# XiYe20/NPVP

Hardware: AMD Instinct MI355X
Metric: predictor train frames/sec (higher is better)
Workload: dtype f32 (two-term fp16 split of amax-scaled operands, 3 MFMAs per product, fp32 accumulate: fp32-grade; small GEMMs: three-term bf16 split)

## Files before the change

### include/npvp_hip.h

```cpp
#ifndef NPVP_HIP_H
#define NPVP_HIP_H
#include <stddef.h>
#ifdef __cplusplus
extern "C" {
#endif

typedef void* npvp_stream_t;

int npvp_version(void);
const char* npvp_last_error(void);
long long npvp_launch_count(void);
void* npvp_stream_create_low_priority(int* least, int* greatest);
int npvp_stream_destroy(void* stream);
void* npvp_event_create(void);
int npvp_event_record(void* event, void* stream);
float npvp_event_elapsed_ms(void* event0, void* event1);
int npvp_event_destroy(void* event);

long long npvp_graph_node_counts(void* graph, long long* counts, long long* memset_bytes, int max_memsets);

long long npvp_gemm_workspace_bytes(int M, int N, int K);
int npvp_gemm_kernel_id(int a_kc, int b_kc, int M, int N, int K, int precision, int has_planes);
int npvp_gemm_route(int a_kc, int b_kc, int M, int N, int K, int precision, int has_planes, int plain_epilogue, int* out4);
int npvp_gemm_f32(int a_kc, int b_kc, int M, int N, int K, const float* A, long long lda, const float* B, long long ldb,
                  float* C, long long ldc, const float* bias, int act, const float* aux_in, float* aux_out,
                  const float* residual, long long ldr, float drop_p, int drop_mode, int drop_g1, int drop_g2,
                  const unsigned long long* seed, unsigned int salt, float alpha, int precision, float* colsum_a,
                  const void* b_pre, int accumulate, float* rowstats, const float* a_amax, const float* b_amax,
                  float* c_amax, unsigned int* range_flag, float adrop_p, int adrop_g1, int adrop_g2, unsigned int adrop_salt,
                  void* workspace, long long ws_bytes, npvp_stream_t stream);
int npvp_frame_stats_finalize(const float* part, int parts_per_frame, float values_per_part, float* mean, float* rstd,
                              int frames, float eps, npvp_stream_t stream);
int npvp_split_weight(const float* w, long long ld, int N, int K, void* F, void* D, npvp_stream_t stream);
int npvp_split_weights_batched(const void* desc, int count, npvp_stream_t stream);
int npvp_amax(const float* x, long long rows, long long cols, long long ld, float* slot, npvp_stream_t stream);

typedef struct npvp_reduce_job {
  const float* ws; float* out; long long ldc; int M, N, splits, accum; float alpha; int blocks; const float* cs_part; float* cs_out;
} npvp_reduce_job_t;
int npvp_wgrad_f16_chainable(int M, int N, int K);
long long npvp_wgrad_f16_chain_workspace_bytes(int M, int N, int K);
int npvp_wgrad_f16_chained(int M, int N, int K, const float* dy, long long lda, const float* x, long long ldb, float* dw,
                           long long ldc, float* db, int accumulate, const float* a_amax, const float* b_amax,
                           unsigned int* range_flag, float adrop_p, int adrop_g1, int adrop_g2, unsigned int adrop_salt,
                           const unsigned long long* seed, const void* prev_job, void* my_job, void* workspace,
                           long long ws_bytes, npvp_stream_t stream);
int npvp_splitk_reduce_job(const void* job, npvp_stream_t stream);
int npvp_splitk_reduce_multi(const void* jobs, int n, npvp_stream_t stream);
int npvp_linear_bwd_f16_takes(int R, int N, int K);
int npvp_linear_bwd_f16(int R, int N, int K, const float* dy, long long ldy, const float* dy_amax, const void* w_planes_d,
                        const float* w_amax, float* dx, long long ldx, int act, const float* aux_in, const float* residual,
                        long long ldr, float drop_p, int drop_mode, int drop_g1, int drop_g2, unsigned int drop_salt, float* dx_amax,
                        const float* x, long long ldxx, const float* x_amax, float* dw, long long ldw, float* db,
                        unsigned int* range_flag, float adrop_p, int adrop_g1, int adrop_g2, unsigned int adrop_salt,
                        const unsigned long long* seed, const void* prev_job, void* my_job, void* workspace, long long ws_bytes,
                        npvp_stream_t stream);
int npvp_split_weight_f16(const float* w, long long ld, int N, int K, void* F, void* D, float* amax_slot, npvp_stream_t stream);
int npvp_split_weights_f16(const void* desc, int count, void* amax_table, long long amax_bytes, npvp_stream_t stream);

int npvp_layernorm_fwd(const float* x, const float* w, const float* b, float* y, float* mean, float* rstd, long long rows,
                       int C, float eps, int relu, float* y_amax, npvp_stream_t stream);
long long npvp_layernorm_bwd_workspace_bytes(long long rows, int C);
int npvp_layernorm_bwd(const float* dy, const float* x, const float* w, const float* b, const float* mean,
                       const float* rstd, float* dx, float* dw, float* db, long long rows, int C, int relu,
                       const float* dres ,
                       int accumulate , float* dx_amax,
                       void* workspace, long long ws_bytes, npvp_stream_t stream);
int npvp_layernorm_bwd_reduce(const void* workspace, float* dw, float* db, long long rows, int C, int accumulate,
                              npvp_stream_t stream);

int npvp_layernorm_bwd_reduce_job(const void* workspace, float* dw, float* db, long long rows, int C, int accumulate, void* job);
int npvp_frameln_act_bwd_reduce_job(const void* workspace, float* dw, float* db, int frames, int per_frame, int accumulate, void* job);
int npvp_mlpdw_mid_bwd_reduce_job(const void* workspace, float* gw, float* gb, int frames, int Ch, void* job);
int npvp_sum_rows_multi(const void* jobs, int n, npvp_stream_t stream);

int npvp_layernorm_nchw_fwd(const float* x, const float* w, const float* b, float* out_nchw, float* mean, float* rstd, int frames,
                            int P, int C, float eps, int relu, npvp_stream_t stream);

int npvp_frame_stats(const float* x, const float* add, float* mean, float* rstd, int frames, int T, int per_frame,
                     float eps, npvp_stream_t stream);
int npvp_posfuse_fwd(const float* x, const float* add, const float* beta, const float* gamma, float* y, float* mean,
                     float* rstd, int N, int T, int per_frame, float eps, float* y_amax, npvp_stream_t stream);
int npvp_ln_posfuse_fwd(const float* x, const float* lw, const float* lb, float ln_eps, float* y1, float* ln_mean, float* ln_rstd,
                        const float* add, const float* beta, const float* gamma, float* fused, float* pf_mean, float* pf_rstd,
                        int N, int T, int P, int C, float pf_eps, float* y1_amax, float* fused_amax, npvp_stream_t stream);
int npvp_posfuse_bwd_fused(int N, int T, int per_frame);
int npvp_posfuse_bwd(const float* dy, const float* x, const float* add, const float* gamma, const float* mean,
                     const float* rstd, float* du, float* dyxh, float* dbeta, float* dgamma, int N, int T, int per_frame,
                     int accumulate, void* workspace, long long ws_bytes , npvp_stream_t stream);

int npvp_posfuse_instance_fwd(const float* x, const float* add, const float* beta, const float* gamma, float* y, float* mean,
                              float* rstd, int N, int T, int P, int C, float eps, float* y_amax, npvp_stream_t stream);
int npvp_posfuse_instance_bwd(const float* dy, const float* x, const float* add, const float* gamma, const float* mean,
                              const float* rstd, float* du, float* dyxh, int N, int T, int P, int C, npvp_stream_t stream);

int npvp_frameln_act_fwd(const float* h, const float* mean, const float* rstd, const float* w, const float* b,
                         const float* res, float* out, int frames, int per_frame, float drop_p, unsigned int salt,
                         float dp_p, unsigned int dp_salt, int frames_per_sample, const unsigned long long* seed,
                         float* out_amax, npvp_stream_t stream);
long long npvp_frameln_act_bwd_workspace_bytes(int frames, int per_frame);
int npvp_frameln_act_bwd(const float* dout, const float* h, const float* mean, const float* rstd, const float* w,
                         const float* b, float* dh, float* dw, float* db, int frames, int per_frame, float drop_p,
                         unsigned int salt, float dp_p, unsigned int dp_salt, int frames_per_sample,
                         const unsigned long long* seed, int accumulate ,
                         float* dh_amax, void* workspace, long long ws_bytes, npvp_stream_t stream);
int npvp_frameln_act_bwd_reduce(const void* workspace, float* dw, float* db, int frames, int per_frame, int accumulate,
                                npvp_stream_t stream);
int npvp_dwconv3x3(const float* a, const float* wt, const float* bias, float* out, int frames, int H, int W, int Ch,
                   int flip, npvp_stream_t stream);
int npvp_dwconv3x3_stats(const float* a, const float* wt, const float* bias, float* out, float* mean, float* rstd, int frames,
                         int H, int W, int Ch, float eps, void* workspace, long long ws_bytes, npvp_stream_t stream);
int npvp_mlpdw_mid_fwd(const float* h1, const float* mean1, const float* rstd1, const float* w1n, const float* b1n,
                       const float* wt, const float* bias, float* h2, float* mean2, float* rstd2, int frames, int H, int W,
                       int Ch, float eps, void* workspace, long long ws_bytes, npvp_stream_t stream);
int npvp_mlpdw_mid_fwd_parts(const float* h1, const float* part1, int J1, float nb1, float* mean1, float* rstd1, const float* w1n,
                             const float* b1n, const float* wt, const float* bias, float* h2, float* part2, int frames, int H,
                             int W, int Ch, float eps, npvp_stream_t stream);
int npvp_frameln_act_fwd_parts(const float* h, const float* part, int J, float nb, float eps, float* mean, float* rstd,
                               const float* w, const float* b, const float* res, float* out, int frames, int per_frame,
                               float drop_p, unsigned int salt, float dp_p, unsigned int dp_salt, int frames_per_sample,
                               const unsigned long long* seed, float* out_amax, npvp_stream_t stream);
long long npvp_mlpdw_mid_bwd_workspace_bytes(int frames, int Ch);
int npvp_mlpdw_mid_bwd(const float* dh2, const float* h1, const float* mean1, const float* rstd1, const float* w1n,
                       const float* b1n, const float* wt, float* da1, float* dwt_db, float* psum, int frames, int H, int W,
                       int Ch, int accumulate, void* workspace, long long ws_bytes, npvp_stream_t stream);
int npvp_mlpdw_mid_bwd_reduce(const void* workspace, float* dwt_db, int frames, int Ch, int accumulate, npvp_stream_t stream);
int npvp_mlpdw_mid_bwd_reduce_into(const void* workspace, float* gw, float* gb, int frames, int Ch, npvp_stream_t stream);
int npvp_mlpdw_mid_bwd_n2(const float* da2, const float* h2, const float* mean2, const float* rstd2, const float* w2n,
                          const float* b2n, const float* psum2, int nparts2, float drop_p, unsigned int salt,
                          const unsigned long long* seed, const float* h1, const float* mean1, const float* rstd1,
                          const float* w1n, const float* b1n, const float* wt, float* da1, float* dwt_db, float* psum, int frames,
                          int H, int W, int Ch, int accumulate, void* workspace, long long ws_bytes, npvp_stream_t stream);
int npvp_frameln_act_bwd_pgrad(const float* dout, const float* h, const float* mean, const float* rstd, const float* w,
                               const float* b, float* psum, float* dw, float* db, int frames, int per_frame, float drop_p,
                               unsigned int salt, float dp_p, unsigned int dp_salt, int frames_per_sample,
                               const unsigned long long* seed, int accumulate, void* workspace, long long ws_bytes,
                               npvp_stream_t stream);
int npvp_frameln_act_bwd_apply(const float* dout, const float* h, const float* mean, const float* rstd, const float* w,
                               const float* b, const float* psum, int nparts, float* dh, float* dw, float* db, int frames,
                               int per_frame, int accumulate, float* dh_amax, void* workspace, long long ws_bytes,
                               npvp_stream_t stream);

int npvp_im2col3x3(const float* in, float* out, int frames, int H, int W, int C, int col2im, npvp_stream_t stream);
long long npvp_dwconv3x3_wgrad_workspace_bytes(int frames, int Ch);
int npvp_dwconv3x3_wgrad(const float* a, const float* dout, float* dwt_db, int frames, int H, int W, int Ch,
                         void* workspace, long long ws_bytes, npvp_stream_t stream);

int npvp_attn_fwd(const float* q, long long ld_q, const float* k, long long ld_k, const float* v, long long ld_v, float* o,
                  long long ld_o, int mode, int dim0, int P, int W, int ws, int Tq, int Tk, int heads, int head_dim,
                  int mask_mode, float drop_p, const unsigned long long* seed, unsigned int salt, float* o_amax,
                  npvp_stream_t stream);
int npvp_attn_bwd(const float* q, long long ld_q, const float* k, long long ld_k, const float* v, long long ld_v,
                  const float* go, long long ld_o, float* dq, long long ld_dq, float* dk, long long ld_dk, float* dv,
                  long long ld_dv, int mode, int dim0, int P, int W, int ws, int Tq, int Tk, int heads, int head_dim,
                  int mask_mode, float drop_p, const unsigned long long* seed, unsigned int salt, float* dq_amax,
                  float* dk_amax , float* dv_amax,
                  npvp_stream_t stream);
int npvp_attn_long_fwd(const float* q, long long ld_q, const float* k, long long ld_k, const float* v, long long ld_v, float* o,
                       long long ld_o, int mode, int dim0, int P, int W, int ws, int Tq, int Tk, int heads, int head_dim,
                       int mask_mode, float drop_p, const unsigned long long* seed, unsigned int salt, float* o_amax,
                       npvp_stream_t stream);
long long npvp_attn_long_bwd_workspace_bytes(int mode, int dim0, int P, int W, int ws, int Tq, int Tk, int heads);
int npvp_attn_long_bwd(const float* q, long long ld_q, const float* k, long long ld_k, const float* v, long long ld_v,
                       const float* go, long long ld_o, float* dq, long long ld_dq, float* dk, long long ld_dk, float* dv,
                       long long ld_dv, int mode, int dim0, int P, int W, int ws, int Tq, int Tk, int heads, int head_dim,
                       int mask_mode, float drop_p, const unsigned long long* seed, unsigned int salt, float* dq_amax,
                       float* dk_amax , float* dv_amax, void* workspace, long long ws_bytes,
                       npvp_stream_t stream);

int npvp_drop_apply(const float* x, float* out, long long rows, int ncols, float p, int mode, int g1, int g2,
                    const unsigned long long* seed, unsigned int salt, float* out_amax, npvp_stream_t stream);
int npvp_transpose(const float* in, float* out, int batch, int R, int C, npvp_stream_t stream);
int npvp_dwtb_accumulate(const float* dwtb, float* gw, float* gb, int C, npvp_stream_t stream);
int npvp_dwtb_build(const float* w, const float* b, float* wtb, int C, npvp_stream_t stream);
int npvp_reduce_mid(const float* in, float* out, int A, int B, long long Cc, float scale, int accumulate, npvp_stream_t stream);
int npvp_broadcast_mid(const float* in, float* out, int A, int B, long long Cc, float scale, npvp_stream_t stream);

long long npvp_colsum_workspace_bytes(long long rows, int N);
int npvp_colsum(const float* x, long long rows, int N, long long ld, float* out, int accumulate ,
                void* workspace, long long ws_bytes, npvp_stream_t stream);

int npvp_l1_mean(const float* a, const float* b, long long n, float lam, float* out, void* workspace, long long ws_bytes,
                 npvp_stream_t stream);
int npvp_l1_mean_bwd(const float* a, const float* b, long long n, const float* gout, float lam, float* da, npvp_stream_t stream);
int npvp_sum_all(const float* x, long long n, float* out, void* workspace, long long ws_bytes, npvp_stream_t stream);

int npvp_grad_norm_clip(const float* g, long long n, float max_norm, float* out2, void* workspace, long long ws_bytes,
                        npvp_stream_t stream);
int npvp_adamw_step(float* p, float* g, float* m, float* v, long long n, const float* hyper, float beta1, float beta2,
                    float eps, float weight_decay, const float* clip, long long clip_begin, long long clip_end,
                    int write_back_grad, npvp_stream_t stream);

long long npvp_sqdiff_workspace_bytes(int N, long long per_image);
int npvp_sqdiff_per_image(const float* x, const float* y, int N, long long per_image, float data_range, float scale, float* out,
                          void* workspace, long long ws_bytes, npvp_stream_t stream);
long long npvp_ssim_workspace_bytes(int N, int C, int H, int W);
int npvp_ssim_per_image(const float* img1, const float* img2, int N, int C, int H, int W, const float* taps ,
                        int window_size, float* out, void* workspace, long long ws_bytes, npvp_stream_t stream);

int npvp_u8hwc_to_f32chw(const void* src_u8, float* dst, long long frames, int H, int W, int C, const float* mean,
                         const float* std, npvp_stream_t stream);

int npvp_bias_act(const float* x, const float* bias, const float* residual, float* out, long long outer, long long inner, int C,
                  int layout, int act, npvp_stream_t stream);
int npvp_act_bwd(const float* g, const float* y, float* dx, long long n, int act, npvp_stream_t stream);

int npvp_bn_workspace_bytes(int C);
int npvp_bn_stats(const float* x, long long outer, long long inner, int C, int layout, double* sums, void* workspace, long long ws_bytes,
                  npvp_stream_t stream);
int npvp_bn_act_apply(const float* x, const float* w, const float* b, const float* residual, const double* sums, long long count,
                      float eps, float momentum, float* running_mean, float* running_var, long long outer, long long inner, int C,
                      int layout, int act, float* y, float* mean, float* rstd, npvp_stream_t stream);
int npvp_bn_act_bwd(const float* g, const float* x, const float* mean, const float* rstd, const float* w, const float* b, long long outer,
                    long long inner, int C, int layout, int act, int train, float* dx, float* dw, float* db, void* workspace,
                    long long ws_bytes, npvp_stream_t stream);
int npvp_bn_act_apply_sync(const float* x, const float* w, const float* b, const float* residual, const double* stat, float eps,
                           float momentum, float* running_mean, float* running_var, long long outer, long long inner, int C, int layout,
                           int act, float* y, float* mean, float* rstd, npvp_stream_t stream);
int npvp_bn_bwd_sums(const float* g, const float* x, const float* mean, const float* rstd, const float* w, const float* b, long long outer,
                     long long inner, int C, int layout, int act, double* sums, float* dw, float* db, void* workspace, long long ws_bytes,
                     npvp_stream_t stream);
int npvp_bn_act_bwd_apply(const float* g, const float* x, const float* mean, const float* rstd, const float* w, const float* b,
                          const double* sums, const double* count, long long outer, long long inner, int C, int layout, int act, float* dx,
                          npvp_stream_t stream);
// ... 26 lines not shown
```

### npvp_amd/_lib.py

```python
import ctypes
import os

_HERE = os.path.dirname(os.path.abspath(__file__))
LIB_PATH = os.path.join(_HERE, "libnpvp_hip.so")

c_int, c_ll, c_f, c_u, c_p = ctypes.c_int, ctypes.c_longlong, ctypes.c_float, ctypes.c_uint, ctypes.c_void_p

SIGNATURES = {
    "npvp_version": (c_int, []),
    "npvp_last_error": (ctypes.c_char_p, []),
    "npvp_launch_count": (c_ll, []),
    "npvp_dp_unique_id": (c_int, [c_p]),
    "npvp_dp_init": (c_int, [c_int, c_int, c_p]),
    "npvp_dp_world": (c_int, []),
    "npvp_dp_rank": (c_int, []),
    "npvp_dp_allreduce_async": (c_int, [c_p, c_ll, c_p]),
    "npvp_dp_wait": (c_int, [c_p]),
    "npvp_dp_finalize": (c_int, []),
    "npvp_stream_create_low_priority": (c_p, [c_p, c_p]),
    "npvp_stream_destroy": (c_int, [c_p]),
    "npvp_event_create": (c_p, []),
    "npvp_event_record": (c_int, [c_p, c_p]),
    "npvp_event_elapsed_ms": (c_f, [c_p, c_p]),
    "npvp_event_destroy": (c_int, [c_p]),
    "npvp_graph_node_counts": (c_ll, [c_p, c_p, c_p, c_int]),
    "npvp_gemm_workspace_bytes": (c_ll, [c_int, c_int, c_int]),
    "npvp_gemm_kernel_id": (c_int, [c_int, c_int, c_int, c_int, c_int, c_int, c_int]),
    "npvp_gemm_route": (c_int, [c_int, c_int, c_int, c_int, c_int, c_int, c_int, c_int, c_p]),
    "npvp_gemm_f32": (c_int, [c_int, c_int, c_int, c_int, c_int, c_p, c_ll, c_p, c_ll, c_p, c_ll, c_p, c_int, c_p, c_p,
                              c_p, c_ll, c_f, c_int, c_int, c_int, c_p, c_u, c_f, c_int, c_p, c_p, c_int, c_p, c_p, c_p, c_p, c_p,
                              c_f, c_int, c_int, c_u, c_p, c_ll, c_p]),
    "npvp_amax": (c_int, [c_p, c_ll, c_ll, c_ll, c_p, c_p]),
    "npvp_wgrad_f16_chainable": (c_int, [c_int, c_int, c_int]),
    "npvp_wgrad_f16_chain_workspace_bytes": (c_ll, [c_int, c_int, c_int]),
    "npvp_wgrad_f16_chained": (c_int, [c_int, c_int, c_int, c_p, c_ll, c_p, c_ll, c_p, c_ll, c_p, c_int, c_p, c_p, c_p, c_f, c_int, c_int,
                                       c_u, c_p, c_p, c_p, c_p, c_ll, c_p]),
    "npvp_splitk_reduce_job": (c_int, [c_p, c_p]),
    "npvp_splitk_reduce_multi": (c_int, [c_p, c_int, c_p]),
    "npvp_linear_bwd_f16_takes": (c_int, [c_int, c_int, c_int]),
    "npvp_linear_bwd_f16": (c_int, [c_int, c_int, c_int, c_p, c_ll, c_p, c_p, c_p, c_p, c_ll, c_int, c_p, c_p, c_ll, c_f, c_int, c_int, c_int,
                                    c_u, c_p, c_p, c_ll, c_p, c_p, c_ll, c_p, c_p, c_f, c_int, c_int, c_u, c_p, c_p, c_p, c_p, c_ll, c_p]),
    "npvp_split_weight_f16": (c_int, [c_p, c_ll, c_int, c_int, c_p, c_p, c_p, c_p]),
    "npvp_split_weights_f16": (c_int, [c_p, c_int, c_p, c_ll, c_p]),
    "npvp_frame_stats_finalize": (c_int, [c_p, c_int, c_f, c_p, c_p, c_int, c_f, c_p]),
    "npvp_split_weight": (c_int, [c_p, c_ll, c_int, c_int, c_p, c_p, c_p]),
    "npvp_split_weights_batched": (c_int, [c_p, c_int, c_p]),
    "npvp_layernorm_fwd": (c_int, [c_p, c_p, c_p, c_p, c_p, c_p, c_ll, c_int, c_f, c_int, c_p, c_p]),
    "npvp_layernorm_bwd_workspace_bytes": (c_ll, [c_ll, c_int]),
    "npvp_layernorm_bwd": (c_int, [c_p, c_p, c_p, c_p, c_p, c_p, c_p, c_p, c_p, c_ll, c_int, c_int, c_p, c_int, c_p, c_p, c_ll, c_p]),
    "npvp_layernorm_bwd_reduce": (c_int, [c_p, c_p, c_p, c_ll, c_int, c_int, c_p]),
    "npvp_layernorm_bwd_reduce_job": (c_int, [c_p, c_p, c_p, c_ll, c_int, c_int, c_p]),
    "npvp_frameln_act_bwd_reduce_job": (c_int, [c_p, c_p, c_p, c_int, c_int, c_int, c_p]),
    "npvp_mlpdw_mid_bwd_reduce_job": (c_int, [c_p, c_p, c_p, c_int, c_int, c_p]),
    "npvp_sum_rows_multi": (c_int, [c_p, c_int, c_p]),
    "npvp_layernorm_nchw_fwd": (c_int, [c_p, c_p, c_p, c_p, c_p, c_p, c_int, c_int, c_int, c_f, c_int, c_p]),
    "npvp_frameln_act_bwd_reduce": (c_int, [c_p, c_p, c_p, c_int, c_int, c_int, c_p]),
    "npvp_frame_stats": (c_int, [c_p, c_p, c_p, c_p, c_int, c_int, c_int, c_f, c_p]),
    "npvp_posfuse_fwd": (c_int, [c_p, c_p, c_p, c_p, c_p, c_p, c_p, c_int, c_int, c_int, c_f, c_p, c_p]),
    "npvp_posfuse_instance_fwd": (c_int, [c_p, c_p, c_p, c_p, c_p, c_p, c_p, c_int, c_int, c_int, c_int, c_f, c_p, c_p]),
    "npvp_posfuse_instance_bwd": (c_int, [c_p, c_p, c_p, c_p, c_p, c_p, c_p, c_p, c_int, c_int, c_int, c_int, c_p]),
    "npvp_ln_posfuse_fwd": (c_int, [c_p, c_p, c_p, c_f, c_p, c_p, c_p, c_p, c_p, c_p, c_p, c_p, c_p, c_int, c_int, c_int, c_int, c_f,
                                    c_p, c_p, c_p]),
    "npvp_posfuse_bwd_fused": (c_int, [c_int, c_int, c_int]),
    "npvp_posfuse_bwd": (c_int, [c_p, c_p, c_p, c_p, c_p, c_p, c_p, c_p, c_p, c_p, c_int, c_int, c_int, c_int, c_p, c_ll, c_p]),
    "npvp_frameln_act_fwd": (c_int, [c_p, c_p, c_p, c_p, c_p, c_p, c_p, c_int, c_int, c_f, c_u, c_f, c_u, c_int, c_p, c_p, c_p]),
    "npvp_frameln_act_bwd_workspace_bytes": (c_ll, [c_int, c_int]),
    "npvp_frameln_act_bwd": (c_int, [c_p, c_p, c_p, c_p, c_p, c_p, c_p, c_p, c_p, c_int, c_int, c_f, c_u, c_f, c_u, c_int,
                                     c_p, c_int, c_p, c_p, c_ll, c_p]),
    "npvp_dwconv3x3": (c_int, [c_p, c_p, c_p, c_p, c_int, c_int, c_int, c_int, c_int, c_p]),
    "npvp_dwconv3x3_stats": (c_int, [c_p, c_p, c_p, c_p, c_p, c_p, c_int, c_int, c_int, c_int, c_f, c_p, c_ll, c_p]),
    "npvp_mlpdw_mid_fwd": (c_int, [c_p, c_p, c_p, c_p, c_p, c_p, c_p, c_p, c_p, c_p, c_int, c_int, c_int, c_int, c_f, c_p, c_ll, c_p]),
    "npvp_mlpdw_mid_fwd_parts": (c_int, [c_p, c_p, c_int, c_f, c_p, c_p, c_p, c_p, c_p, c_p, c_p, c_p, c_int, c_int, c_int, c_int, c_f, c_p]),
    "npvp_frameln_act_fwd_parts": (c_int, [c_p, c_p, c_int, c_f, c_f, c_p, c_p, c_p, c_p, c_p, c_p, c_int, c_int, c_f, c_u, c_f, c_u, c_int,
                                           c_p, c_p, c_p]),
    "npvp_mlpdw_mid_bwd_workspace_bytes": (c_ll, [c_int, c_int]),
    "npvp_mlpdw_mid_bwd": (c_int, [c_p, c_p, c_p, c_p, c_p, c_p, c_p, c_p, c_p, c_p, c_int, c_int, c_int, c_int, c_int, c_p, c_ll, c_p]),
    "npvp_mlpdw_mid_bwd_reduce": (c_int, [c_p, c_p, c_int, c_int, c_int, c_p]),
    "npvp_mlpdw_mid_bwd_reduce_into": (c_int, [c_p, c_p, c_p, c_int, c_int, c_p]),
    "npvp_mlpdw_mid_bwd_n2": (c_int, [c_p, c_p, c_p, c_p, c_p, c_p, c_p, c_int, c_f, c_u, c_p, c_p, c_p, c_p, c_p, c_p, c_p, c_p, c_p,
                                      c_p, c_int, c_int, c_int, c_int, c_int, c_p, c_ll, c_p]),
    "npvp_frameln_act_bwd_pgrad": (c_int, [c_p, c_p, c_p, c_p, c_p, c_p, c_p, c_p, c_p, c_int, c_int, c_f, c_u, c_f, c_u, c_int,
                                           c_p, c_int, c_p, c_ll, c_p]),
    "npvp_frameln_act_bwd_apply": (c_int, [c_p, c_p, c_p, c_p, c_p, c_p, c_p, c_int, c_p, c_p, c_p, c_int, c_int, c_int, c_p, c_p, c_ll, c_p]),
    "npvp_im2col3x3": (c_int, [c_p, c_p, c_int, c_int, c_int, c_int, c_int, c_p]),
    "npvp_dwconv3x3_wgrad_workspace_bytes": (c_ll, [c_int, c_int]),
    "npvp_dwconv3x3_wgrad": (c_int, [c_p, c_p, c_p, c_int, c_int, c_int, c_int, c_p, c_ll, c_p]),
    "npvp_attn_fwd": (c_int, [c_p, c_ll, c_p, c_ll, c_p, c_ll, c_p, c_ll, c_int, c_int, c_int, c_int, c_int, c_int, c_int,
                              c_int, c_int, c_int, c_f, c_p, c_u, c_p, c_p]),
    "npvp_attn_bwd": (c_int, [c_p, c_ll, c_p, c_ll, c_p, c_ll, c_p, c_ll, c_p, c_ll, c_p, c_ll, c_p, c_ll, c_int, c_int,
                              c_int, c_int, c_int, c_int, c_int, c_int, c_int, c_int, c_f, c_p, c_u, c_p, c_p, c_p, c_p]),
    "npvp_attn_long_fwd": (c_int, [c_p, c_ll, c_p, c_ll, c_p, c_ll, c_p, c_ll, c_int, c_int, c_int, c_int, c_int, c_int, c_int,
                                   c_int, c_int, c_int, c_f, c_p, c_u, c_p, c_p]),
    "npvp_attn_long_bwd_workspace_bytes": (c_ll, [c_int, c_int, c_int, c_int, c_int, c_int, c_int, c_int]),
    "npvp_attn_long_bwd": (c_int, [c_p, c_ll, c_p, c_ll, c_p, c_ll, c_p, c_ll, c_p, c_ll, c_p, c_ll, c_p, c_ll, c_int, c_int,
                                   c_int, c_int, c_int, c_int, c_int, c_int, c_int, c_int, c_f, c_p, c_u, c_p, c_p, c_p, c_p, c_ll, c_p]),
    "npvp_drop_apply": (c_int, [c_p, c_p, c_ll, c_int, c_f, c_int, c_int, c_int, c_p, c_u, c_p, c_p]),
    "npvp_transpose": (c_int, [c_p, c_p, c_int, c_int, c_int, c_p]),
    "npvp_dwtb_accumulate": (c_int, [c_p, c_p, c_p, c_int, c_p]),
    "npvp_dwtb_build": (c_int, [c_p, c_p, c_p, c_int, c_p]),
    "npvp_reduce_mid": (c_int, [c_p, c_p, c_int, c_int, c_ll, c_f, c_int, c_p]),
    "npvp_broadcast_mid": (c_int, [c_p, c_p, c_int, c_int, c_ll, c_f, c_p]),
    "npvp_colsum_workspace_bytes": (c_ll, [c_ll, c_int]),
    "npvp_colsum": (c_int, [c_p, c_ll, c_int, c_ll, c_p, c_int, c_p, c_ll, c_p]),
    "npvp_grad_norm_clip": (c_int, [c_p, c_ll, c_f, c_p, c_p, c_ll, c_p]),
    "npvp_l1_mean": (c_int, [c_p, c_p, c_ll, c_f, c_p, c_p, c_ll, c_p]),
    "npvp_l1_mean_bwd": (c_int, [c_p, c_p, c_ll, c_p, c_f, c_p, c_p]),
    "npvp_sum_all": (c_int, [c_p, c_ll, c_p, c_p, c_ll, c_p]),
    "npvp_adamw_step": (c_int, [c_p, c_p, c_p, c_p, c_ll, c_p, c_f, c_f, c_f, c_f, c_p, c_ll, c_ll, c_int, c_p]),
    "npvp_sqdiff_workspace_bytes": (c_ll, [c_int, c_ll]),
    "npvp_sqdiff_per_image": (c_int, [c_p, c_p, c_int, c_ll, c_f, c_f, c_p, c_p, c_ll, c_p]),
    "npvp_ssim_workspace_bytes": (c_ll, [c_int, c_int, c_int, c_int]),
    "npvp_u8hwc_to_f32chw": (c_int, [c_p, c_p, c_ll, c_int, c_int, c_int, c_p, c_p, c_p]),
    "npvp_bias_act": (c_int, [c_p, c_p, c_p, c_p, c_ll, c_ll, c_int, c_int, c_int, c_p]),
    "npvp_act_bwd": (c_int, [c_p, c_p, c_p, c_ll, c_int, c_p]),
    "npvp_bn_workspace_bytes": (c_int, [c_int]),
    "npvp_bn_stats": (c_int, [c_p, c_ll, c_ll, c_int, c_int, c_p, c_p, c_ll, c_p]),
    "npvp_bn_act_apply": (c_int, [c_p, c_p, c_p, c_p, c_p, c_ll, c_f, c_f, c_p, c_p, c_ll, c_ll, c_int, c_int, c_int, c_p, c_p, c_p, c_p]),
    "npvp_bn_act_bwd": (c_int, [c_p, c_p, c_p, c_p, c_p, c_p, c_ll, c_ll, c_int, c_int, c_int, c_int, c_p, c_p, c_p, c_p, c_ll, c_p]),
    "npvp_bn_act_apply_sync": (c_int, [c_p, c_p, c_p, c_p, c_p, c_f, c_f, c_p, c_p, c_ll, c_ll, c_int, c_int, c_int, c_p, c_p, c_p, c_p]),
    "npvp_bn_bwd_sums": (c_int, [c_p, c_p, c_p, c_p, c_p, c_p, c_ll, c_ll, c_int, c_int, c_int, c_p, c_p, c_p, c_p, c_ll, c_p]),
    "npvp_bn_act_bwd_apply": (c_int, [c_p, c_p, c_p, c_p, c_p, c_p, c_p, c_p, c_ll, c_ll, c_int, c_int, c_int, c_p, c_p]),
    "npvp_reflect_pad": (c_int, [c_p, c_p, c_int, c_int, c_int, c_int, c_int, c_int, c_int, c_p]),
    "npvp_nonlocal_attn_fwd": (c_int, [c_p, c_ll, c_p, c_ll, c_p, c_ll, c_p, c_ll, c_p, c_int, c_int, c_int, c_int, c_int, c_p]),
    "npvp_nonlocal_attn_bwd": (c_int, [c_p, c_ll, c_p, c_ll, c_p, c_ll, c_p, c_ll, c_p, c_p, c_p, c_ll, c_p, c_ll, c_p, c_ll, c_int, c_int,
                                       c_int, c_int, c_int, c_p]),
    "npvp_nonlocal_attn_grid_fwd": (c_int, [c_p, c_ll, c_p, c_ll, c_p, c_ll, c_p, c_ll, c_p, c_int, c_int, c_int, c_int, c_int, c_p]),
    "npvp_nonlocal_attn_grid_bwd": (c_int, [c_p, c_ll, c_p, c_ll, c_p, c_ll, c_p, c_ll, c_p, c_p, c_p, c_ll, c_p, c_ll, c_p, c_ll, c_int,
                                            c_int, c_int, c_int, c_int, c_p]),
    "npvp_ssim_per_image": (c_int, [c_p, c_p, c_int, c_int, c_int, c_int, c_p, c_int, c_p, c_p, c_ll, c_p]),
}

_lib = None


def lib():
    global _lib
    if _lib is None:
        if not os.path.exists(LIB_PATH):
            raise RuntimeError(
                f"{LIB_PATH} is missing - the HIP extension has not been built. Run "
                "`python -c 'import __graft_entry__ as g; g.build()'` (or `python npvp_amd/build.py`). "
                "npvp_amd has no CPU fallback.")
        L = ctypes.CDLL(LIB_PATH, mode=os.RTLD_NOW)
        bound = _Bound()
        for name, (res, args) in SIGNATURES.items():
            fn = getattr(L, name)
            fn.restype, fn.argtypes = res, args
            setattr(bound, name, fn)
        bound._cdll = L
        bound._fast = 0
        if os.environ.get("NPVP_FASTCALL", "1") == "1":
            try:
                from . import _npvp_fast as F
            except ImportError as e:
                import warnings
                warnings.warn(f"npvp_amd._npvp_fast is not built ({e}): every call goes through ctypes (same kernels, more host time)")
            else:
                for name in SIGNATURES:
                    f = getattr(F, name, None)
                    if f is not None:
                        setattr(bound, name, f)
                        bound._fast += 1
        _lib = bound
    return _lib


# ... 9 lines not shown
```

### npvp_amd/csrc/gemm.h

```cpp
#pragma once
#include <type_traits>
#include "common.h"

namespace npvp {

typedef float f32x16 __attribute__((ext_vector_type(16)));
typedef __bf16 bf16x8 __attribute__((ext_vector_type(8)));
typedef __bf16 bf16x4 __attribute__((ext_vector_type(4)));

struct ReduceJob {
  const float* ws; float* out; long long ldc; int M, N, splits, accum; float alpha; int blocks; const float* cs_part; float* cs_out;
};

struct GemmParams {
  const float* A; const float* B; float* C;
  const float* bias;
  const float* residual;
  float* aux_out;
  const float* aux_in;
  float* rowstats;
  float* colsum;
  const unsigned long long* seed;
  long long lda, ldb, ldc, ldr;
  int M, N, K;
  int act;
  DropSpec drop;
  DropSpec adrop;
  int tiles_m, tiles_n;
  int splits;
  float alpha;
  const void* b_pre;
  long long b_pre_plane;
  int colgroups;
  int accum;
  const float* a_amax; const float* b_amax; float* c_amax;
  unsigned int* range_flag;
  ReduceJob prev;
};

__device__ __forceinline__ void splitk_reduce_body(const ReduceJob& j, int bid, int nblocks, float& cmax) {
  const long long total4 = (long long)j.M * j.N / 4, cs4 = j.cs_out ? j.M / 4 : 0;
  for (long long i = (long long)bid * 256 + threadIdx.x; i < total4 + cs4; i += (long long)nblocks * 256) {
    if (i >= total4) {
      const long long e = (i - total4) * 4;
      float4 s = make_float4(0.f, 0.f, 0.f, 0.f);
      for (int zz = 0; zz < j.splits; ++zz) {
        const float4 v = ld4(j.cs_part + (long long)zz * j.M + e);
        s.x += v.x; s.y += v.y; s.z += v.z; s.w += v.w;
      }
      if (j.accum) { const float4 o = ld4(j.cs_out + e); s.x += o.x; s.y += o.y; s.z += o.z; s.w += o.w; }
      st4(j.cs_out + e, s);
      continue;
    }
    const long long e = i * 4;
    const int m = (int)(e / j.N), n = (int)(e - (long long)m * j.N);
    float4 s = make_float4(0.f, 0.f, 0.f, 0.f);
    for (int zz = 0; zz < j.splits; ++zz) {
      const float4 v = ld4(j.ws + (long long)zz * j.M * j.N + e);
      s.x += v.x; s.y += v.y; s.z += v.z; s.w += v.w;
    }
    s.x *= j.alpha; s.y *= j.alpha; s.z *= j.alpha; s.w *= j.alpha;
    if (j.accum) { const float4 o = ld4(j.out + (long long)m * j.ldc + n); s.x += o.x; s.y += o.y; s.z += o.z; s.w += o.w; }
    st4(j.out + (long long)m * j.ldc + n, s);
    cmax = amax4(cmax, s);
  }
}

__device__ __forceinline__ void store_colsum(const GemmParams& p, long long idx, float v) {
  p.colsum[idx] = (p.accum && p.splits == 1) ? p.colsum[idx] + v : v;
}

constexpr int EPI_LD = 36;
constexpr int EPI_FLOATS = 32 * EPI_LD;

__device__ __forceinline__ void epi_transpose(const f32x16& acc, float* scr, int lane, float4 (&v)[4]) {
  const int r = lane & 31, h = lane >> 5;
#pragma unroll
  for (int g = 0; g < 16; ++g) scr[(((g & 3) + 8 * (g >> 2)) + 4 * h) * EPI_LD + r] = acc[g];
  const int rr = lane >> 3, cq = lane & 7;
#pragma unroll
  for (int k = 0; k < 4; ++k) v[k] = *reinterpret_cast<const float4*>(scr + (rr + 8 * k) * EPI_LD + 4 * cq);
}

__device__ __forceinline__ float4 f4_mad(const float4& a, float s, const float4& b) {
  return make_float4(a.x * s + b.x, a.y * s + b.y, a.z * s + b.z, a.w * s + b.w);
}
__device__ __forceinline__ void f4_add(float4& a, const float4& b) { a.x += b.x; a.y += b.y; a.z += b.z; a.w += b.w; }

template <int I, int N, class F>
__device__ __forceinline__ void static_for(F&& f) {
  if constexpr (I < N) {
    f(std::integral_constant<int, I>{});
    static_for<I + 1, N>(f);
  }
}

__device__ __forceinline__ float4 epilogue_row_scales(const GemmParams& p, unsigned long long seed, int row0, int lane) {
  float4 sc = make_float4(1.f, 1.f, 1.f, 1.f);
  if (p.drop.thresh && p.drop.mode != 0) {
    const int r = row0 + (lane >> 3);
    sc.x = drop_spec_scale(p.drop, seed, r, 0, 1); sc.y = drop_spec_scale(p.drop, seed, r + 8, 0, 1);
    sc.z = drop_spec_scale(p.drop, seed, r + 16, 0, 1); sc.w = drop_spec_scale(p.drop, seed, r + 24, 0, 1);
  }
  return sc;
}

template <bool CHECK>
__device__ __forceinline__ void epilogue_rows(const GemmParams& p, float4 (&v)[4], int row0, int col0, int lane, int z,
                                              unsigned long long seed, float& cmax, float4 rowsc, float alpha) {
  const int rb = row0 + (lane >> 3), col = col0 + 4 * (lane & 7);
// ... 206 lines not shown
```

### npvp_amd/csrc/gemm.hip

```cpp
#include "gemm.h"
#include "partials.h"
#include <type_traits>

namespace npvp {

constexpr int BM = 128, BN = 128, BK = 32, GEMM_THREADS = 256;

template <bool KC> struct Stager;

template <> struct Stager<true> {
  static constexpr int LD = 129;
  float4 r[4];
  __device__ __forceinline__ void load(const float* src, long long ld, int row0, int nrows, int k0) {
    const int t = threadIdx.x;
    const int kc = (t & 7) * 4;
#pragma unroll
    for (int i = 0; i < 4; ++i) {
      const int row = row0 + (t >> 3) + 32 * i;
      r[i] = (row < nrows) ? ld4(src + (long long)row * ld + k0 + kc) : make_float4(0.f, 0.f, 0.f, 0.f);
    }
  }
  __device__ __forceinline__ void store(float* s) const {
    const int t = threadIdx.x;
    const int kc = (t & 7) * 4;
// ... 413 lines not shown
  NPVP_CHECK_ARG(N > 0 && K > 0 && N % 8 == 0 && K % 8 == 0 && ld % 4 == 0, "split_weight: N, K must be multiples of 8");
  NPVP_CHECK_ARG(((uintptr_t)w % 16) == 0, "split_weight: w must be 16-byte aligned");
  const long long total = (long long)N * K / 8;
  int blocks = (int)((total + 255) / 256); if (blocks > 4096) blocks = 4096;
  if (F) { NPVP_LAUNCH(split_weight_fwd_kernel, dim3(blocks), dim3(256), 0, stream, w, ld, N, K, (__bf16*)F); NPVP_CHECK_LAUNCH(); }
  if (D) { NPVP_LAUNCH(split_weight_dgrad_kernel, dim3(blocks), dim3(256), 0, stream, w, ld, N, K, (__bf16*)D); NPVP_CHECK_LAUNCH(); }
  return NPVP_OK;
}

extern "C" int npvp_split_weights_batched(const void* desc, int count, hipStream_t stream) {
  NPVP_CHECK_ARG(desc && count > 0, "split_weights_batched: empty table");
  NPVP_LAUNCH(split_weights_batched_kernel, dim3(128, count), dim3(256), 0, stream, (const SplitDesc*)desc);
  NPVP_CHECK_LAUNCH();
  return NPVP_OK;
}

struct GemmFacts {
  int a_kc, b_kc, M, N, K, precision;
  bool planes;
  bool plain;
  bool amax;
  bool rowstats;
  long long ws_bytes;
};
struct GemmPlan {
  int id, variant, splits, steps;
  bool planes;
};

static GemmPlan plan_gemm(const GemmFacts& f) {
  const int M = f.M, N = f.N, K = f.K;
  const bool want_h = f.precision == 6;
  const int precision = want_h ? 4 : f.precision;
  int s128 = pick_splits(M, N, K);
  if (s128 > 1 && (!f.plain || f.ws_bytes < npvp_gemm_workspace_bytes(M, N, K))) s128 = 1;
  const bool planes_ok = f.planes && f.a_kc && K % 16 == 0 && N % 8 == 0;
  const bool wgrad = !f.a_kc && !f.b_kc && f.plain && !f.rowstats;
  auto fits = [&](int s) { return s == 1 || (s > 1 && f.ws_bytes >= splitk_workspace_bytes(s, M, N)); };
  GemmPlan pl = {precision == 0 ? 0 : 1, 0, s128, 0, false};
  int v = 0, s = 0;
  if (want_h && planes_ok && f.amax && (v = gemm_f16_variant(M, N, K)) != 0) {
    pl.id = v == 1 ? 5 : 7; pl.variant = v; pl.splits = 1; pl.planes = true;
  } else if (want_h && wgrad && f.amax && fits(s = f16_wgrad_splits(M, N, K))) {
    pl.id = 6; pl.splits = s;
  } else if (!want_h && precision == 4 && planes_ok && s128 == 1 && (v = wide_variant(M, N, K)) != 0) {
    pl.id = v == 1 ? 2 : 4; pl.variant = v; pl.planes = true;
  } else if (precision == 4 && wgrad && fits(s = wide_wgrad_splits(M, N, K))) {
    pl.id = 3; pl.splits = s;
  } else {
    pl.planes = !want_h && precision == 4 && planes_ok && s128 == 1 && !f.rowstats;
  }
  pl.steps = K / pl.splits / (precision == 0 ? BK : 16);
  return pl;
}

static GemmPlan plan_query(int a_kc, int b_kc, int M, int N, int K, int precision, int has_planes, bool plain) {
  return plan_gemm(GemmFacts{a_kc, b_kc, M, N, K, precision, has_planes != 0, plain, true, false, npvp_gemm_workspace_bytes(M, N, K)});
}

extern "C" int npvp_gemm_kernel_id(int a_kc, int b_kc, int M, int N, int K, int precision, int has_planes) {
  return plan_query(a_kc, b_kc, M, N, K, precision, has_planes, true).id;
}

extern "C" int npvp_gemm_route(int a_kc, int b_kc, int M, int N, int K, int precision, int has_planes, int plain_epilogue, int* out4) {
  NPVP_CHECK_ARG(out4 && M > 0 && N > 0 && K > 0, "gemm_route: empty problem or no result array");
  NPVP_CHECK_ARG(precision == 0 || precision == 4 || precision == 5 || precision == 6, "gemm_route: precision must be 0, 4, 5 or 6");
  NPVP_CHECK_ARG(K % BK == 0 && M % 4 == 0 && N % 4 == 0 && !(a_kc == 0 && b_kc == 1), "gemm_route: not a problem npvp_gemm_f32 accepts");
  const GemmPlan r = plan_query(a_kc, b_kc, M, N, K, precision, has_planes, plain_epilogue != 0);
  out4[0] = r.id; out4[1] = r.variant; out4[2] = r.splits; out4[3] = r.steps;
  return NPVP_OK;
}

static int finish_splitk(const GemmParams& p, float* C, long long ldc, float* colsum_a, hipStream_t stream) {
  const long long total4 = (long long)p.M * p.N / 4;
  int blocks = (int)((total4 + 255) / 256); if (blocks > 2048) blocks = 2048;
  const bool cs_here = colsum_a && ((uintptr_t)colsum_a % 16) == 0;
  NPVP_LAUNCH(splitk_reduce_kernel, dim3(blocks), dim3(256), 0, stream, (const float*)p.C, C, p.M, p.N, ldc, p.splits, p.alpha,
              p.accum, cs_here ? (const float*)p.colsum : nullptr, cs_here ? colsum_a : nullptr, p.c_amax);
  NPVP_CHECK_LAUNCH();
  if (!colsum_a || cs_here) return NPVP_OK;
  return finish_partials(make_partials(p.colsum, 0, p.splits, p.splits, p.M, colsum_a, p.accum).job, 0, stream, "gemm: column-sum reduce launch failed");
}

extern "C" int npvp_gemm_f32(int a_kc, int b_kc, int M, int N, int K, const float* A, long long lda, const float* B,
                             long long ldb, float* C, long long ldc, const float* bias, int act, const float* aux_in,
                             float* aux_out, const float* residual, long long ldr, float drop_p, int drop_mode,
                             int drop_g1, int drop_g2, const unsigned long long* seed, unsigned int salt, float alpha,
                             int precision, float* colsum_a, const void* b_pre, int accumulate, float* rowstats,
                             const float* a_amax, const float* b_amax, float* c_amax, unsigned int* range_flag,
                             float adrop_p, int adrop_g1, int adrop_g2, unsigned int adrop_salt,
                             void* workspace, long long ws_bytes, hipStream_t stream) {
  NPVP_CHECK_ARG(M > 0 && N > 0 && K > 0, "gemm: empty problem");
  NPVP_CHECK_ARG(precision == 0 || precision == 4 || precision == 5 || precision == 6,
                 "gemm: precision must be 0 (exact fp32-input MFMA), 4 (three-term bf16 split, 6 MFMAs per product: "
                 "fp32-grade), 5 (two-term bf16 split, 3 MFMAs per product, ~2^-16) or 6 (two-term fp16 split with amax-scaled "
                 "operands, 3 MFMAs per product: fp32-grade; shapes it does not take run as 4)");
  const bool want_h = precision == 6;
  NPVP_CHECK_ARG(K % BK == 0, "gemm: K must be a multiple of 32");
  NPVP_CHECK_ARG(M % 4 == 0 && N % 4 == 0, "gemm: M and N must be multiples of 4");
  NPVP_CHECK_ARG(((uintptr_t)A % 16) == 0 && ((uintptr_t)B % 16) == 0 && ((uintptr_t)C % 16) == 0, "gemm: pointers must be 16-byte aligned");
  NPVP_CHECK_ARG(lda % 4 == 0 && ldb % 4 == 0, "gemm: lda/ldb must be multiples of 4 floats");
  NPVP_CHECK_ARG(ldc % 4 == 0 && (!residual || (ldr % 4 == 0 && ((uintptr_t)residual % 16) == 0)) && (!bias || ((uintptr_t)bias % 16) == 0) &&
                 (!aux_in || ((uintptr_t)aux_in % 16) == 0) && (!aux_out || ((uintptr_t)aux_out % 16) == 0),
                 "gemm: ldc / ldr must be multiples of 4 floats and bias / aux / residual 16-byte aligned (float4 epilogue)");
  NPVP_CHECK_ARG(!(a_kc == 0 && b_kc == 1), "gemm: (a_kc=0,b_kc=1) is not used by the path");
  NPVP_CHECK_ARG((act != 3 && act != 4) || aux_in, "gemm: act 3/4 need aux_in");
  NPVP_CHECK_ARG(drop_p >= 0.f && drop_p < 1.f, "gemm: dropout p out of range");
  NPVP_CHECK_ARG(drop_p == 0.f || seed, "gemm: dropout needs a device seed");
  NPVP_CHECK_ARG(!colsum_a || a_kc == 0, "gemm: colsum_a is the column sum of a [K][M] operand (a_kc = 0)");
  NPVP_CHECK_ARG(!b_pre || ((uintptr_t)b_pre % 16) == 0, "gemm: b_pre must be 16-byte aligned");

  NPVP_CHECK_ARG(adrop_p >= 0.f && adrop_p < 0.5f, "gemm: adrop_p must be in [0, 0.5) (the masked operand must stay inside its amax scale)");
  NPVP_CHECK_ARG(adrop_p == 0.f || (seed && want_h && adrop_g1 > 0 && adrop_g2 > 0 && (a_kc || adrop_g1 % 16 == 0)),
                 "gemm: adrop needs precision 6, a device seed and (for a weight gradient) groups of a multiple of 16 rows");
  NPVP_CHECK_ARG(!rowstats || ((precision == 4 || want_h) && a_kc && b_kc && M % 64 == 0 && N % 128 == 0 && act == 0 && !aux_out && !residual &&
                               drop_p == 0.f && !accumulate),
                 "gemm: rowstats needs the default (bf16x6) forward layout, M % 64 == 0, N % 128 == 0 and a bias-only epilogue");

  const bool plain = !bias && act == 0 && !aux_out && !residual && drop_p == 0.f;
  const GemmPlan plan = plan_gemm(GemmFacts{a_kc, b_kc, M, N, K, precision, b_pre != nullptr, plain,
                                            a_amax && b_amax, rowstats != nullptr, workspace ? ws_bytes : 0});
  NPVP_CHECK_ARG(adrop_p == 0.f || plan.id >= 5, "gemm: adrop was requested but this shape does not run on the fp16 kernels (npvp_gemm_kernel_id tells)");

  GemmParams p;
  p.A = A; p.B = B; p.bias = bias; p.residual = residual; p.aux_out = aux_out; p.aux_in = aux_in;
  p.seed = seed; p.lda = lda; p.ldb = ldb; p.ldr = ldr; p.M = M; p.N = N; p.act = act;
  p.drop = make_drop_spec(drop_p, salt, drop_mode, drop_g1, drop_g2);
  p.adrop = make_drop_spec(adrop_p, adrop_salt, 1, adrop_g1, adrop_g2);
  p.alpha = alpha;
  p.rowstats = rowstats;
  p.a_amax = a_amax; p.b_amax = b_amax; p.c_amax = c_amax; p.range_flag = range_flag;
  p.prev = ReduceJob{};
  p.accum = accumulate ? 1 : 0;
  p.b_pre = plan.planes ? b_pre : nullptr;
  p.b_pre_plane = (long long)N * K;
  p.splits = plan.splits;
  if (plan.splits > 1) aim_at_workspace(p, K, plan.splits, workspace, colsum_a != nullptr);
  else { p.K = K; p.C = C; p.ldc = ldc; p.colsum = colsum_a; }
  p.tiles_m = (M + BM - 1) / BM; p.tiles_n = (N + BN - 1) / BN;
  p.colgroups = (plan.id <= 1 && plan.splits == 1) ? pick_colgroups((long long)N * K * 4, p.tiles_m, p.tiles_n) : 1;

  const dim3 grid(p.tiles_m * p.tiles_n, plan.splits), block(GEMM_THREADS);
  switch (plan.id) {
    case 5: case 7: launch_gemm_f16(p, plan.variant, stream); break;
    case 6: launch_gemm_wgrad_f16(p, stream); break;
    case 2: case 4: launch_gemm_wide(p, plan.variant, stream); break;
    case 3: launch_gemm_wgrad_wide(p, stream); break;
    case 0:
      if (a_kc && b_kc) NPVP_LAUNCH((gemm_f32_kernel<true, true>), grid, block, 0, stream, p);
      else if (a_kc) NPVP_LAUNCH((gemm_f32_kernel<true, false>), grid, block, 0, stream, p);
      else NPVP_LAUNCH((gemm_f32_kernel<false, false>), grid, block, 0, stream, p);
      break;
    default:
      if (precision == 5) {
        if (a_kc && b_kc) NPVP_LAUNCH((gemm_split_db_kernel<2, true, true, false>), grid, block, 0, stream, p);
        else if (a_kc) NPVP_LAUNCH((gemm_split_db_kernel<2, true, false, false>), grid, block, 0, stream, p);
        else NPVP_LAUNCH((gemm_split_db_kernel<2, false, false, false>), grid, block, 0, stream, p);
      } else if (rowstats) NPVP_LAUNCH((gemm_split_db_kernel<3, true, true, false, true>), grid, block, 0, stream, p);
      else if (plan.planes) NPVP_LAUNCH((gemm_split_db_kernel<3, true, true, true>), grid, block, 0, stream, p);
      else if (a_kc && b_kc) NPVP_LAUNCH((gemm_split_db_kernel<3, true, true, false>), grid, block, 0, stream, p);
      else if (a_kc) NPVP_LAUNCH((gemm_split_db_kernel<3, true, false, false>), grid, block, 0, stream, p);
      else NPVP_LAUNCH((gemm_split_db_kernel<3, false, false, false>), grid, block, 0, stream, p);
  }
  NPVP_CHECK_LAUNCH();
  return plan.splits > 1 ? finish_splitk(p, C, ldc, colsum_a, stream) : NPVP_OK;
}
```

### npvp_amd/csrc/gemm_f16.hip

```cpp
#include "gemm.h"
#include <cstdlib>

namespace npvp {

typedef _Float16 f16x8 __attribute__((ext_vector_type(8)));
typedef _Float16 f16x4 __attribute__((ext_vector_type(4)));
typedef __attribute__((address_space(1))) const void* gptr_t;
typedef __attribute__((address_space(3))) void* lptr_t;
typedef float f32x4 __attribute__((ext_vector_type(4)));

__device__ __forceinline__ void split_f16_scaled(const f32x4 v, const float s, f16x4& hi, f16x4& lo) {
  unsigned int h01, h23, l01, l23;
  asm("v_fma_mixlo_f16 %0, %1, %2, 0" : "=v"(h01) : "v"(v[0]), "v"(s));
  asm("v_fma_mixlo_f16 %0, %1, %2, 0" : "=v"(h23) : "v"(v[2]), "v"(s));
  asm("v_fma_mixhi_f16 %0, %1, %2, 0" : "+v"(h01) : "v"(v[1]), "v"(s));
  asm("v_fma_mixhi_f16 %0, %1, %2, 0" : "+v"(h23) : "v"(v[3]), "v"(s));
  asm("v_fma_mixlo_f16 %0, %1, %2, -%3 op_sel_hi:[0,0,1]" : "=v"(l01) : "v"(v[0]), "v"(s), "v"(h01));
  asm("v_fma_mixlo_f16 %0, %1, %2, -%3 op_sel_hi:[0,0,1]" : "=v"(l23) : "v"(v[2]), "v"(s), "v"(h23));
  asm("v_fma_mixhi_f16 %0, %1, %2, -%3 op_sel:[0,0,1] op_sel_hi:[0,0,1]" : "+v"(l01) : "v"(v[1]), "v"(s), "v"(h01));
  asm("v_fma_mixhi_f16 %0, %1, %2, -%3 op_sel:[0,0,1] op_sel_hi:[0,0,1]" : "+v"(l23) : "v"(v[3]), "v"(s), "v"(h23));
  typedef unsigned int u32x2 __attribute__((ext_vector_type(2)));
  const u32x2 hp = {h01, h23}, lp = {l01, l23};
  hi = __builtin_bit_cast(f16x4, hp);
  lo = __builtin_bit_cast(f16x4, lp);
// ... 23 lines not shown
__device__ __forceinline__ void gemm_f16_body(const GemmParams& p, char* lds, const int bid, const int nwg) {
  constexpr int NW = WM * WN, THREADS = 64 * NW;
  constexpr int BM = WM * TM * 32, BN = WN * TN * 32;
  constexpr int APASS = BM / (THREADS / 4);
  static_assert((APASS == 1 || APASS == 2) && BN % 64 == 0, "A staging: a thread stages one or two rows of the tile");
  constexpr int KGS_A = BM * 16 + 64, A_PLANE = 2 * KGS_A, A_BYTES = 2 * A_PLANE;
  constexpr int KGS_B = BN * 16, B_PLANE = 2 * KGS_B, B_BYTES = 2 * B_PLANE;
  constexpr int STAGE = A_BYTES + B_BYTES;
  constexpr int CPS = BN / 64;
  constexpr int NCHUNK = 4 * CPS, CPW = (NCHUNK + NW - 1) / NW;
  static_assert(NST == 2 || NST == 3, "two or three LDS stages");
  static_assert(gemm_f16_lds_bytes<TM, TN, WM, WN, NST>() >= NST * STAGE, "lds size formula");

  int tile_m, tile_n;
  tile_of_block_unsplit(p, nwg, bid, tile_m, tile_n);
  const int m0 = tile_m * BM, n0 = tile_n * BN;
  const int t = threadIdx.x, lane = t & 63, wave = __builtin_amdgcn_readfirstlane(t >> 6);
  const int wm = wave / WN, wn = wave % WN, r = lane & 31, h = lane >> 5;
  const int nk = p.K >> 4;
  const float sa = amax_scale(amax_slot_read(p.a_amax));
  const unsigned int cpeek = amax_peek_block(p.c_amax);

  f32x16 acc[TM][TN];

  const int quad = t & 3, rl = t >> 2;
  const char* a_base = reinterpret_cast<const char*>(p.A + (long long)m0 * p.lda);
  const unsigned int a_off0 = (unsigned int)(((long long)(min(m0 + rl, p.M - 1) - m0) * p.lda + 4 * quad) * 4);
  const unsigned int a_off1 = (unsigned int)(((long long)(min(m0 + rl + BM / 2, p.M - 1) - m0) * p.lda + 4 * quad) * 4);
  const int a_dst = (quad >> 1) * KGS_A + (quad & 1) * 8 + rl * 16;
  float sa0 = sa, sa1 = sa;
  if (p.adrop.thresh) {
    const unsigned long long aseed = *p.seed;
    sa0 *= drop_spec_scale(p.adrop, aseed, min(m0 + rl, p.M - 1), 0, 1);
    sa1 *= drop_spec_scale(p.adrop, aseed, min(m0 + rl + BM / 2, p.M - 1), 0, 1);
  }
  const char* b_base = reinterpret_cast<const char*>(p.b_pre);
  unsigned int b_off[CPW];
  int b_dst[CPW];
#pragma unroll
  for (int i = 0; i < CPW; ++i) {
    const int c = wave + NW * i;
    const int slab = c / CPS, part = c - slab * CPS, s = slab >> 1, kg = slab & 1;
    const int col = min(n0 + part * 64 + lane, p.N - 1);
    b_off[i] = (unsigned int)(((long long)s * (p.b_pre_plane >> 3) + (long long)kg * p.N + col) * 16);
    b_dst[i] = A_BYTES + s * B_PLANE + kg * KGS_B + part * 1024;
  }
  const long long b_step = 32ll * p.N;
  const unsigned int lds_u32 = (unsigned int)(size_t)((lptr_t)lds);

  const int fa_off = h * KGS_A + (wm * TM * 32 + r) * 16;
  const int fb_off = A_BYTES + h * KGS_B + (wn * TN * 32 + r) * 16;

  f32x4 ea0, ea1 = {0.f, 0.f, 0.f, 0.f}, eb0, eb1 = {0.f, 0.f, 0.f, 0.f};
#define NPVP_H_ALOAD(R0, R1, KT)                                                                           \
  { const char* ab_ = a_base + ((long long)min((KT), nk - 1) << 6);                                        \
    asm volatile("global_load_dwordx4 %0, %1, %2" : "=v"(R0) : "v"(a_off0), "s"(ab_) : "memory");          \
    if constexpr (APASS == 2) asm volatile("global_load_dwordx4 %0, %1, %2" : "=v"(R1) : "v"(a_off1), "s"(ab_) : "memory"); }
#define NPVP_H_WAIT_BUT_NEWEST(...)                                                                        \
  { if constexpr (APASS == 2) asm volatile("s_waitcnt vmcnt(2) lgkmcnt(0)" : __VA_ARGS__ :: "memory");     \
    else asm volatile("s_waitcnt vmcnt(1) lgkmcnt(0)" : __VA_ARGS__ :: "memory"); }
#define NPVP_H_WAIT_BUT_THIS_STEP(...)                                                                     \
  asm volatile("s_waitcnt vmcnt(%2) lgkmcnt(0)" : __VA_ARGS__ : "n"(CPW + APASS) : "memory");
#define NPVP_H_ASTORE(ST, V, ROWOFF)                                                     \
  { if (ROWOFF) rm1 = fmaxf(fmaxf(rm1, fmaxf(fabsf((V)[0]), fabsf((V)[1]))), fmaxf(fabsf((V)[2]), fabsf((V)[3])));  \
    else rm0 = fmaxf(fmaxf(rm0, fmaxf(fabsf((V)[0]), fabsf((V)[1]))), fmaxf(fabsf((V)[2]), fabsf((V)[3])));         \
    f16x4 hi_, lo_; split_f16_scaled((V), (ROWOFF) ? sa1 : sa0, hi_, lo_);               \
    *reinterpret_cast<f16x4*>((ST) + a_dst + (ROWOFF)) = hi_;                            \
    *reinterpret_cast<f16x4*>((ST) + A_PLANE + a_dst + (ROWOFF)) = lo_; }
#define NPVP_H_BLOAD(ST, KT)                                                             \
  { const char* bb_ = b_base + (long long)min((KT), nk - 1) * b_step;                    \
    _Pragma("unroll") for (int i_ = 0; i_ < CPW; ++i_)                                   \
      if (NCHUNK % NW == 0 || wave + NW * i_ < NCHUNK) {                                 \
        const unsigned int m0_ = lds_u32 + (unsigned int)((ST) - lds) + (unsigned int)b_dst[i_];          \
        asm volatile("s_mov_b32 m0, %0\n\ts_nop 0\n\tglobal_load_lds_dwordx4 %1, %2"                     \
                     :: "s"(m0_), "v"(b_off[i_]), "s"(bb_) : "memory", "m0"); } }
  static_assert(NCHUNK % NW == 0, "the hand-counted waits assume CPW LDS-DMA pieces per wave and step");

  __shared__ int guard_flags[NW];
  float rm0 = 0.f, rm1 = 0.f;
  bool rescued = false;
  const float zrow = 1.f;
  float rf0 = zrow, rf1 = zrow;
  const f32x16 zero16 = {0.f, 0.f, 0.f, 0.f, 0.f, 0.f, 0.f, 0.f, 0.f, 0.f, 0.f, 0.f, 0.f, 0.f, 0.f, 0.f};
  auto run_tile = [&]() __attribute__((always_inline)) {
  NPVP_H_BLOAD(lds, 0)
  NPVP_H_ALOAD(ea0, ea1, 0)
  asm volatile("s_waitcnt vmcnt(0)" : "+v"(ea0), "+v"(ea1) :: "memory");
  NPVP_H_ASTORE(lds, ea0, 0)
  if constexpr (APASS == 2) NPVP_H_ASTORE(lds, ea1, (BM / 2) * 16)
  if constexpr (NST == 3) NPVP_H_BLOAD(lds + STAGE, 1)
  NPVP_H_ALOAD(ea0, ea1, 1)
  NPVP_H_ALOAD(eb0, eb1, 2)
  NPVP_H_WAIT_BUT_NEWEST("+v"(ea0), "+v"(ea1))
  __builtin_amdgcn_s_barrier();

#define NPVP_H_STEP(KT, CUR, NXT, R0, R1, RN0, RN1) NPVP_H_STEP_(KT, CUR, NXT, NXT, R0, R1, RN0, RN1, false)
#define NPVP_H_STEP3(KT, CUR, NXT, B2, R0, R1, RN0, RN1) NPVP_H_STEP_(KT, CUR, NXT, B2, R0, R1, RN0, RN1, false)
#define NPVP_H_STEP_(KT, CUR, NXT, B2, R0, R1, RN0, RN1, FIRST)                                            \
  {                                                                                                        \
    const char* st_ = lds + (CUR) * STAGE;                                                                 \
    char* nx_ = lds + (NXT) * STAGE;                                                                       \
    NPVP_H_BLOAD(lds + (B2) * STAGE, (KT) + (NST - 1))                                                     \
    f16x8 fb_[2][TN];                                                                                      \
    _Pragma("unroll") for (int s_ = 0; s_ < 2; ++s_)                                                       \
      _Pragma("unroll") for (int j_ = 0; j_ < TN; ++j_)                                                    \
        fb_[s_][j_] = *reinterpret_cast<const f16x8*>(st_ + fb_off + s_ * B_PLANE + j_ * 512);             \
    _Pragma("unroll") for (int i_ = 0; i_ < TM; ++i_) {                                                    \
      f16x8 fa_[2];                                                                                        \
      _Pragma("unroll") for (int s_ = 0; s_ < 2; ++s_)                                                     \
        fa_[s_] = *reinterpret_cast<const f16x8*>(st_ + fa_off + s_ * A_PLANE + i_ * 512);                 \
      if (i_ == 0) { NPVP_H_ASTORE(nx_, R0, 0) if constexpr (APASS == 2) NPVP_H_ASTORE(nx_, R1, (BM / 2) * 16) } \
      if (i_ == TM - 1) { NPVP_H_ALOAD(R0, R1, (KT) + 3) }                                                 \
                                                                                 \
      _Pragma("unroll") for (int j_ = 0; j_ < TN; ++j_) acc[i_][j_] = __builtin_amdgcn_mfma_f32_32x32x16_f16(fa_[1], fb_[0][j_], (FIRST) ? zero16 : acc[i_][j_], 0, 0, 0); \
      _Pragma("unroll") for (int j_ = 0; j_ < TN; ++j_) acc[i_][j_] = __builtin_amdgcn_mfma_f32_32x32x16_f16(fa_[0], fb_[1][j_], acc[i_][j_], 0, 0, 0); \
      _Pragma("unroll") for (int j_ = 0; j_ < TN; ++j_) acc[i_][j_] = __builtin_amdgcn_mfma_f32_32x32x16_f16(fa_[0], fb_[0][j_], acc[i_][j_], 0, 0, 0); \
    }                                                                                                      \
    __builtin_amdgcn_sched_barrier(0);        \
    if constexpr (NST == 3) { NPVP_H_WAIT_BUT_THIS_STEP("+v"(RN0), "+v"(RN1)) }                            \
    else { NPVP_H_WAIT_BUT_NEWEST("+v"(RN0), "+v"(RN1)) }                                                  \
    __builtin_amdgcn_s_barrier();                                                                          \
  }

  if constexpr (NST == 2) {
  NPVP_H_STEP_(0, 0, 1, 1, ea0, ea1, eb0, eb1, true)
  int kt = 1;
  for (; kt + 1 < nk; kt += 2) {
    NPVP_H_STEP(kt, 1, 0, eb0, eb1, ea0, ea1)
    NPVP_H_STEP(kt + 1, 0, 1, ea0, ea1, eb0, eb1)
  }
  if (kt < nk) NPVP_H_STEP(kt, 1, 0, eb0, eb1, ea0, ea1)
  } else {
  NPVP_H_STEP_(0, 0, 1, 2, ea0, ea1, eb0, eb1, true)
  int kt = 1;
  for (; kt + 5 < nk; kt += 6) {
    NPVP_H_STEP3(kt, 1, 2, 0, eb0, eb1, ea0, ea1)
    NPVP_H_STEP3(kt + 1, 2, 0, 1, ea0, ea1, eb0, eb1)
    NPVP_H_STEP3(kt + 2, 0, 1, 2, eb0, eb1, ea0, ea1)
    NPVP_H_STEP3(kt + 3, 1, 2, 0, ea0, ea1, eb0, eb1)
    NPVP_H_STEP3(kt + 4, 2, 0, 1, eb0, eb1, ea0, ea1)
    NPVP_H_STEP3(kt + 5, 0, 1, 2, ea0, ea1, eb0, eb1)
  }
  if (kt < nk) NPVP_H_STEP3(kt, 1, 2, 0, eb0, eb1, ea0, ea1)
  if (kt + 1 < nk) NPVP_H_STEP3(kt + 1, 2, 0, 1, ea0, ea1, eb0, eb1)
  if (kt + 2 < nk) NPVP_H_STEP3(kt + 2, 0, 1, 2, eb0, eb1, ea0, ea1)
  if (kt + 3 < nk) NPVP_H_STEP3(kt + 3, 1, 2, 0, ea0, ea1, eb0, eb1)
  if (kt + 4 < nk) NPVP_H_STEP3(kt + 4, 2, 0, 1, eb0, eb1, ea0, ea1)
  }
  asm volatile("s_waitcnt vmcnt(0)" : "+v"(ea0), "+v"(ea1), "+v"(eb0), "+v"(eb1) :: "memory");
  if constexpr (NST == 3) __builtin_amdgcn_s_barrier();
  };
  run_tile();
  {
    rm0 = fmaxf(rm0, __shfl_xor(rm0, 1)); rm0 = fmaxf(rm0, __shfl_xor(rm0, 2));
    rm1 = fmaxf(rm1, __shfl_xor(rm1, 1)); rm1 = fmaxf(rm1, __shfl_xor(rm1, 2));
    const int et = (int)((__float_as_uint(sa) >> 23) & 0xffu);
    const int e0 = (int)((__float_as_uint(rm0) >> 23) & 0xffu), e1 = (int)((__float_as_uint(rm1) >> 23) & 0xffu);
    const int d0 = 268 - et - e0, d1 = 268 - et - e1;
    const bool ok0 = e0 >= 16 && e0 != 255 && d0 > 0 && d0 <= 120, ok1 = e1 >= 16 && e1 != 255 && d1 > 0 && d1 <= 120;
    if (block_any<NW>((ok0 && d0 >= 18) || (ok1 && d1 >= 18), guard_flags, wave)) {
      const float g0 = sa0 * pow2_recip(sa), g1 = sa1 * pow2_recip(sa);
      rf0 = ok0 ? __uint_as_float((unsigned int)(127 - d0) << 23) : 1.f;
      rf1 = ok1 ? __uint_as_float((unsigned int)(127 - d1) << 23) : 1.f;
      sa0 = (ok0 ? amax_scale(rm0) : sa) * g0;
      sa1 = (ok1 ? amax_scale(rm1) : sa) * g1;
      rescued = true;
// ... 596 lines not shown
```

### npvp_amd/csrc/norm.hip

```cpp
#include "partials.h"
#include <cstring>
#include <cstdlib>

namespace npvp {

template <int NV>
__global__ __launch_bounds__(256) void ln_fwd_kernel(const float* __restrict__ x, const float* __restrict__ w,
                                                     const float* __restrict__ b, float* __restrict__ y,
                                                     float* __restrict__ mean, float* __restrict__ rstd, long long rows,
                                                     float eps, int relu, float* __restrict__ amax) {
  constexpr int C = NV * 256;
  __shared__ float ared[4];
  const unsigned int peek = amax_peek_block(amax);
  const int lane = threadIdx.x & 63;
  float4 ww[NV], bb[NV];
#pragma unroll
  for (int i = 0; i < NV; ++i) { ww[i] = ld4(w + (i * 64 + lane) * 4); bb[i] = ld4(b + (i * 64 + lane) * 4); }
  float am = 0.f;
  for (long long row = (long long)blockIdx.x * 4 + (threadIdx.x >> 6); row < rows; row += (long long)gridDim.x * 4) {
    float4 v[NV];
    float s = 0.f;
#pragma unroll
    for (int i = 0; i < NV; ++i) {
      v[i] = ld4(x + row * C + (i * 64 + lane) * 4);
// ... 447 lines not shown
  }
  if (dbeta) {
    if (accum) { const float4 o = ld4(dbeta + (long long)t * per_frame + e); sb.x += o.x; sb.y += o.y; sb.z += o.z; sb.w += o.w; }
    st4(dbeta + (long long)t * per_frame + e, sb);
  }
  if (dgamma) {
    if (accum) { const float4 o = ld4(dgamma + (long long)t * per_frame + e); sg.x += o.x; sg.y += o.y; sg.z += o.z; sg.w += o.w; }
    st4(dgamma + (long long)t * per_frame + e, sg);
  }
}

constexpr int PFI_MAXP = 64;
__global__ __launch_bounds__(256) void posfuse_inst_fwd_kernel(const float* __restrict__ x, const float* __restrict__ add,
                                                               const float* __restrict__ beta, const float* __restrict__ gamma,
                                                               float* __restrict__ y, float* __restrict__ mean,
                                                               float* __restrict__ rstd, int T, int P, int C, float eps,
                                                               float* __restrict__ amax) {
  __shared__ float ared[4];
  const unsigned int peek = amax_peek_block(amax);
  const int c = blockIdx.x * blockDim.x + threadIdx.x;
  const long long f = blockIdx.y;
  float am = 0.f;
  if (c < C) {
    const int n = (int)(f / T), t = (int)(f - (long long)n * T);
    const float* xp = x + f * P * C + c;
    const float* ap = add ? add + (long long)n * P * C + c : nullptr;
    float u[PFI_MAXP], s = 0.f;
#pragma unroll
    for (int p = 0; p < PFI_MAXP; ++p) if (p < P) { u[p] = xp[(long long)p * C] + (ap ? ap[(long long)p * C] : 0.f); s += u[p]; }
    const float mu = s / P;
    float q = 0.f;
#pragma unroll
    for (int p = 0; p < PFI_MAXP; ++p) if (p < P) { const float d = u[p] - mu; q += d * d; }
    const float rs = rsqrtf(q / P + eps);
    mean[f * C + c] = mu; rstd[f * C + c] = rs;
    const float* bp = beta + (long long)t * P * C + c;
    const float* gp = gamma ? gamma + (long long)t * P * C + c : nullptr;
#pragma unroll
    for (int p = 0; p < PFI_MAXP; ++p) if (p < P) {
      float o = (u[p] - mu) * rs;
      if (gp) o *= 1.f + gp[(long long)p * C];
      o += bp[(long long)p * C];
      y[f * P * C + (long long)p * C + c] = o;
      am = fmaxf(am, fabsf(o));
    }
  }
  amax_slot_commit_block(amax, am, ared, peek);
}

__global__ __launch_bounds__(256) void posfuse_inst_bwd_kernel(const float* __restrict__ dy, const float* __restrict__ x,
                                                               const float* __restrict__ add, const float* __restrict__ gamma,
                                                               const float* __restrict__ mean, const float* __restrict__ rstd,
                                                               float* __restrict__ du, float* __restrict__ dyxh, int T, int P,
                                                               int C) {
  const int c = blockIdx.x * blockDim.x + threadIdx.x;
  const long long f = blockIdx.y;
  if (c >= C) return;
  const int n = (int)(f / T), t = (int)(f - (long long)n * T);
  const long long base = f * P * C + c;
  const float* ap = add ? add + (long long)n * P * C + c : nullptr;
  const float* gp = gamma ? gamma + (long long)t * P * C + c : nullptr;
  const float mu = mean[f * C + c], rs = rstd[f * C + c];
  float g[PFI_MAXP], uh[PFI_MAXP], s1 = 0.f, s2 = 0.f;
#pragma unroll
  for (int p = 0; p < PFI_MAXP; ++p) if (p < P) {
    const float d = dy[base + (long long)p * C];
    uh[p] = (x[base + (long long)p * C] + (ap ? ap[(long long)p * C] : 0.f) - mu) * rs;
    if (dyxh) dyxh[base + (long long)p * C] = d * uh[p];
    g[p] = gp ? d * (1.f + gp[(long long)p * C]) : d;
    s1 += g[p]; s2 += g[p] * uh[p];
  }
  s1 /= P; s2 /= P;
#pragma unroll
  for (int p = 0; p < PFI_MAXP; ++p) if (p < P) du[base + (long long)p * C] = rs * (g[p] - s1 - uh[p] * s2);
}

struct FlnParams {
  const float* h; const float* mean; const float* rstd; const float* w; const float* b;
  const float* res;
  const unsigned long long* seed;
  unsigned int drop_thresh; float drop_inv_keep; unsigned int salt;
  unsigned int dp_thresh; float dp_inv_keep; unsigned int dp_salt; int frames_per_sample;
  int per_frame; long long total4;
};

__device__ __forceinline__ float fln_frame_scale(const FlnParams& p, unsigned long long seed, long long f) {
  if (!p.dp_thresh) return 1.f;
  return drop_scale(seed, p.dp_salt, (unsigned long long)((unsigned int)f / (unsigned int)p.frames_per_sample), p.dp_thresh, p.dp_inv_keep);
}
__device__ __forceinline__ float fln_scale(const FlnParams& p, unsigned long long seed, float frame_scale, long long gidx) {
  if (!p.drop_thresh) return frame_scale;
  return drop_scale(seed, p.salt, (unsigned long long)gidx, p.drop_thresh, p.drop_inv_keep) * frame_scale;
}

__global__ void frameln_act_fwd_kernel(FlnParams p, float* __restrict__ out, float* __restrict__ amax) {
  const int pf4 = p.per_frame / 4;
  __shared__ float ared[16];
  const unsigned int peek = amax_peek_block(amax);
  float am = 0.f;
  const unsigned long long seed = (p.seed && (p.drop_thresh || p.dp_thresh)) ? *p.seed : 0ull;
  for (long long i = (long long)blockIdx.x * blockDim.x + threadIdx.x; i < p.total4; i += (long long)gridDim.x * blockDim.x) {
    const long long f = i / pf4;
    const int e = (int)(i - f * pf4) * 4;
    const float mu = p.mean[f], rs = p.rstd[f];
    const float fsc = fln_frame_scale(p, seed, f);
    const float4 v = ld4(p.h + f * p.per_frame + e), ww = ld4(p.w + e), bb = ld4(p.b + e);
    const long long g0 = f * p.per_frame + e;
    float4 o;
    o.x = gelu_f((v.x - mu) * rs * ww.x + bb.x) * fln_scale(p, seed, fsc, g0 + 0);
    o.y = gelu_f((v.y - mu) * rs * ww.y + bb.y) * fln_scale(p, seed, fsc, g0 + 1);
    o.z = gelu_f((v.z - mu) * rs * ww.z + bb.z) * fln_scale(p, seed, fsc, g0 + 2);
    o.w = gelu_f((v.w - mu) * rs * ww.w + bb.w) * fln_scale(p, seed, fsc, g0 + 3);
    if (p.res) { const float4 r = ld4(p.res + g0); o.x += r.x; o.y += r.y; o.z += r.z; o.w += r.w; }
    st4(out + g0, o);
    am = amax4(am, o);
  }
  amax_slot_commit_block(amax, am, ared, peek);
}

__global__ __launch_bounds__(256) void frameln_act_fwd_parts_kernel(FlnParams p, const float* __restrict__ part, int J, float nb,
                                                                    float eps, float* __restrict__ mean_out,
                                                                    float* __restrict__ rstd_out, float* __restrict__ out,
                                                                    float* __restrict__ amax) {
  __shared__ float ared[16];
  const unsigned int peek = amax_peek_block(amax);
  const int bpf = p.per_frame / 4096;
  const long long f = blockIdx.x / bpf;
  const int e0 = (blockIdx.x - (int)f * bpf) * 4096;
  const unsigned long long seed = (p.seed && (p.drop_thresh || p.dp_thresh)) ? *p.seed : 0ull;
  float mu, rs;
  frame_stats_merge(part, f, J, nb, eps, mu, rs);
  if (e0 == 0 && threadIdx.x == 0) { mean_out[f] = mu; rstd_out[f] = rs; }
  const float fsc = fln_frame_scale(p, seed, f);
  float am = 0.f;
#pragma unroll
  for (int k = 0; k < 4; ++k) {
    const int e = e0 + (k * 256 + threadIdx.x) * 4;
    const long long g0 = f * p.per_frame + e;
    const float4 v = ld4(p.h + g0), ww = ld4(p.w + e), bb = ld4(p.b + e);
    float4 o;
    o.x = gelu_f((v.x - mu) * rs * ww.x + bb.x) * fln_scale(p, seed, fsc, g0 + 0);
    o.y = gelu_f((v.y - mu) * rs * ww.y + bb.y) * fln_scale(p, seed, fsc, g0 + 1);
    o.z = gelu_f((v.z - mu) * rs * ww.z + bb.z) * fln_scale(p, seed, fsc, g0 + 2);
    o.w = gelu_f((v.w - mu) * rs * ww.w + bb.w) * fln_scale(p, seed, fsc, g0 + 3);
    if (p.res) { const float4 r = ld4(p.res + g0); o.x += r.x; o.y += r.y; o.z += r.z; o.w += r.w; }
    st4(out + g0, o);
    am = amax4(am, o);
  }
  amax_slot_commit_block(amax, am, ared, peek);
}

constexpr int FLN_PARTS = 4;
__global__ __launch_bounds__(512) void frameln_act_bwd_stats_kernel(FlnParams p, const float* __restrict__ dout,
                                                                    float* __restrict__ psum) {
  __shared__ float red[8];
  const long long f = blockIdx.x;
  const unsigned long long seed = (p.seed && (p.drop_thresh || p.dp_thresh)) ? *p.seed : 0ull;
  const float mu = p.mean[f], rs = p.rstd[f];
  const float fsc = fln_frame_scale(p, seed, f);
  float s1 = 0.f, s2 = 0.f;
  const int span = p.per_frame / FLN_PARTS, e0 = blockIdx.y * span, e1 = blockIdx.y == FLN_PARTS - 1 ? p.per_frame : e0 + span;
  for (int e = e0 + threadIdx.x * 4; e < e1; e += 512 * 4) {
    const long long g0 = f * p.per_frame + e;
    const float4 v = ld4(p.h + g0), ww = ld4(p.w + e), bb = ld4(p.b + e), d = ld4(dout + g0);
    const float hx = (v.x - mu) * rs, hy = (v.y - mu) * rs, hz = (v.z - mu) * rs, hw = (v.w - mu) * rs;
    const float gx = d.x * fln_scale(p, seed, fsc, g0 + 0) * gelu_grad_f(hx * ww.x + bb.x) * ww.x;
    const float gy = d.y * fln_scale(p, seed, fsc, g0 + 1) * gelu_grad_f(hy * ww.y + bb.y) * ww.y;
    const float gz = d.z * fln_scale(p, seed, fsc, g0 + 2) * gelu_grad_f(hz * ww.z + bb.z) * ww.z;
    const float gw = d.w * fln_scale(p, seed, fsc, g0 + 3) * gelu_grad_f(hw * ww.w + bb.w) * ww.w;
    s1 += gx + gy + gz + gw;
    s2 += gx * hx + gy * hy + gz * hz + gw * hw;
  }
  s1 = block_sum<8>(s1, red);
  s2 = block_sum<8>(s2, red);
  if (threadIdx.x == 0) { psum[(f * FLN_PARTS + blockIdx.y) * 2] = s1; psum[(f * FLN_PARTS + blockIdx.y) * 2 + 1] = s2; }
}

__global__ void frameln_act_bwd_fused_kernel(FlnParams p, const float* __restrict__ dout, const float* __restrict__ psum,
                                             float* __restrict__ dh, float* __restrict__ part, int frames,
                                             int frames_per_chunk, int nparts, float* __restrict__ amax) {
  const int e = (blockIdx.x * blockDim.x + threadIdx.x) * 4;
  __shared__ float ared[16];
  const unsigned int peek = amax_peek_block(amax);
  float am = 0.f;
  if (e >= p.per_frame) { amax_slot_commit_block(amax, am, ared, peek); return; }
  const unsigned long long seed = (p.seed && (p.drop_thresh || p.dp_thresh)) ? *p.seed : 0ull;
  const float4 ww = ld4(p.w + e), bb = ld4(p.b + e);
  float4 aw = make_float4(0.f, 0.f, 0.f, 0.f), ab = make_float4(0.f, 0.f, 0.f, 0.f);
  const int f0 = blockIdx.y * frames_per_chunk;
  const int f1 = min(frames, f0 + frames_per_chunk);
  for (long long f = f0; f < f1; ++f) {
    const long long g0 = f * p.per_frame + e;
    const float mu = p.mean[f], rs = p.rstd[f];
    const float fsc = fln_frame_scale(p, seed, f);
    float a1 = 0.f, a2 = 0.f;
    for (int j = 0; j < nparts; ++j) { a1 += psum[(f * nparts + j) * 2]; a2 += psum[(f * nparts + j) * 2 + 1]; }
    a1 /= p.per_frame; a2 /= p.per_frame;
    const float4 v = ld4(p.h + g0), d = ld4(dout + g0);
    const float hx = (v.x - mu) * rs, hy = (v.y - mu) * rs, hz = (v.z - mu) * rs, hw = (v.w - mu) * rs;
    const float dx_ = d.x * fln_scale(p, seed, fsc, g0 + 0) * gelu_grad_f(hx * ww.x + bb.x);
    const float dy_ = d.y * fln_scale(p, seed, fsc, g0 + 1) * gelu_grad_f(hy * ww.y + bb.y);
    const float dz_ = d.z * fln_scale(p, seed, fsc, g0 + 2) * gelu_grad_f(hz * ww.z + bb.z);
    const float dw_ = d.w * fln_scale(p, seed, fsc, g0 + 3) * gelu_grad_f(hw * ww.w + bb.w);
    aw.x += dx_ * hx; aw.y += dy_ * hy; aw.z += dz_ * hz; aw.w += dw_ * hw;
    ab.x += dx_; ab.y += dy_; ab.z += dz_; ab.w += dw_;
    float4 o;
    o.x = rs * (dx_ * ww.x - a1 - hx * a2); o.y = rs * (dy_ * ww.y - a1 - hy * a2);
    o.z = rs * (dz_ * ww.z - a1 - hz * a2); o.w = rs * (dw_ * ww.w - a1 - hw * a2);
    st4(dh + g0, o);
    am = amax4(am, o);
  }
  amax_slot_commit_block(amax, am, ared, peek);
  float* o = part + (long long)blockIdx.y * 2 * p.per_frame;
  st4(o + e, aw);
  st4(o + p.per_frame + e, ab);
}

__global__ __launch_bounds__(256) void frameln_act_bwd_pgrad_kernel(FlnParams p, const float* __restrict__ dout,
                                                                    float* __restrict__ psum, float* __restrict__ part, int frames,
                                                                    int frames_per_chunk) {
  __shared__ float red[4];
  const int e = (blockIdx.x * blockDim.x + threadIdx.x) * 4;
  const int nblk = gridDim.x;
  const unsigned long long seed = (p.seed && (p.drop_thresh || p.dp_thresh)) ? *p.seed : 0ull;
  const float4 ww = ld4(p.w + e), bb = ld4(p.b + e);
  float4 aw = make_float4(0.f, 0.f, 0.f, 0.f), ab = make_float4(0.f, 0.f, 0.f, 0.f);
  const int f0 = blockIdx.y * frames_per_chunk;
  const int f1 = min(frames, f0 + frames_per_chunk);
  for (long long f = f0; f < f1; ++f) {
    const long long g0 = f * p.per_frame + e;
    const float mu = p.mean[f], rs = p.rstd[f];
    const float fsc = fln_frame_scale(p, seed, f);
    const float4 v = ld4(p.h + g0), d = ld4(dout + g0);
    const float hx = (v.x - mu) * rs, hy = (v.y - mu) * rs, hz = (v.z - mu) * rs, hw = (v.w - mu) * rs;
    const float dx_ = d.x * fln_scale(p, seed, fsc, g0 + 0) * gelu_grad_f(hx * ww.x + bb.x);
    const float dy_ = d.y * fln_scale(p, seed, fsc, g0 + 1) * gelu_grad_f(hy * ww.y + bb.y);
    const float dz_ = d.z * fln_scale(p, seed, fsc, g0 + 2) * gelu_grad_f(hz * ww.z + bb.z);
    const float dw_ = d.w * fln_scale(p, seed, fsc, g0 + 3) * gelu_grad_f(hw * ww.w + bb.w);
    aw.x += dx_ * hx; aw.y += dy_ * hy; aw.z += dz_ * hz; aw.w += dw_ * hw;
    ab.x += dx_; ab.y += dy_; ab.z += dz_; ab.w += dw_;
    const float gx = dx_ * ww.x, gy = dy_ * ww.y, gz = dz_ * ww.z, gw = dw_ * ww.w;
    const float s1 = block_sum<4>((gx + gy) + (gz + gw), red);
    const float s2 = block_sum<4>((gx * hx + gy * hy) + (gz * hz + gw * hw), red);
    if (threadIdx.x == 0) { psum[(f * nblk + blockIdx.x) * 2] = s1; psum[(f * nblk + blockIdx.x) * 2 + 1] = s2; }
  }
  float* o = part + (long long)blockIdx.y * 2 * p.per_frame;
  st4(o + e, aw);
  st4(o + p.per_frame + e, ab);
}

struct SumRowsPlan { int cw, threads; };
static SumRowsPlan plan_sum_rows(const SumRowsJob& q) {
  if (q.mode == 0 && q.nb < 64 && q.ncols >= 4096 && q.ncols % 4 == 0 && q.stride % 4 == 0 && (!q.out_b || q.split % 4 == 0)
      && ((uintptr_t)q.in & 15) == 0)
    return {sum_rows_wide_cols(), 1024};
  if (q.nb >= 64 && q.ncols <= 8192) return {16, 1024};
  return {64, q.nb >= 64 ? 1024 : 256};
}

int launch_sum_rows(const SumRowsJob& q, hipStream_t stream) {
  if (q.mode != 0) return NPVP_ERR_ARG;
  const SumRowsPlan pl = plan_sum_rows(q);
  const auto kernel = pl.cw == sum_rows_wide_cols() ? sum_rows_wide_kernel : pl.cw == 16 ? sum_rows_kernel<16> : sum_rows_kernel<64>;
  NPVP_LAUNCH(kernel, dim3((q.ncols + pl.cw - 1) / pl.cw), dim3(pl.threads), 0, stream, q.in, q.out, q.nb, q.stride, q.ncols, q.accum,
              q.out_b, q.out_b ? q.split : 0);
  return hipGetLastError() == hipSuccess ? NPVP_OK : NPVP_ERR_LAUNCH;
}

struct SumRowsBatch { SumRowsJob j[SRJ_MAX]; int first[SRJ_MAX + 1]; int cw[SRJ_MAX]; int n; };

__global__ __launch_bounds__(1024) void sum_rows_multi_kernel(SumRowsBatch b) {
  __shared__ float red[1024];
  int lo = 0, hi = b.n - 1;
  while (lo < hi) { const int mid = (lo + hi + 1) >> 1; if (b.first[mid] <= (int)blockIdx.x) lo = mid; else hi = mid - 1; }
  const SumRowsJob& J = b.j[lo];
  const int CW = b.cw[lo], sh = CW == 16 ? 4 : 6;
  if (CW == sum_rows_wide_cols()) {
    sum_rows_wide(J.in, J.out, J.out_b, J.nb, J.stride, J.ncols, J.out_b ? J.split : 0, J.accum,
                  (((int)blockIdx.x - b.first[lo]) * 1024 + (int)threadIdx.x) * 4);
    return;
  }
  const int cx = threadIdx.x & (CW - 1), rl = threadIdx.x >> sh, nrl = 1024 >> sh;
  const int c = ((int)blockIdx.x - b.first[lo]) * CW + cx;
  float s = 0.f;
  if (c < J.ncols)
    for (int r = rl; r < J.nb; r += nrl) s += J.in[(long long)r * J.stride + c];
  red[rl * CW + cx] = s;
  __syncthreads();
  if (rl == 0 && c < J.ncols) {
    float t = 0.f;
    for (int i = 0; i < nrl; ++i) t += red[i * CW + cx];
    float* o;
    if (J.mode == 1) { const int tap = c / J.split, ch = c - tap * J.split; o = tap < 9 ? J.out + ch * 9 + tap : J.out_b + ch; }
    else o = (J.out_b && c >= J.split) ? J.out_b + (c - J.split) : J.out + c;
    *o = J.accum ? *o + t : t;
  }
}

static inline int ew_blocks(long long total, int threads) {
  long long b = (total + threads - 1) / threads;
  if (b > 4096) b = 4096;
  if (b < 1) b = 1;
  return (int)b;
}

static void fill_fln(FlnParams& p, const float* h, const float* mean, const float* rstd, const float* w, const float* b,
                     const float* res, int frames, int per_frame, float drop_p, unsigned int salt, float dp_p,
                     unsigned int dp_salt, int frames_per_sample, const unsigned long long* seed) {
  p.h = h; p.mean = mean; p.rstd = rstd; p.w = w; p.b = b; p.res = res; p.seed = seed;
  p.drop_thresh = drop_p > 0.f ? drop_threshold(drop_p) : 0u;
  p.drop_inv_keep = drop_p > 0.f ? 1.f / (1.f - drop_p) : 1.f;
  p.salt = salt;
  p.dp_thresh = dp_p > 0.f ? drop_threshold(dp_p) : 0u;
  p.dp_inv_keep = dp_p > 0.f ? 1.f / (1.f - dp_p) : 1.f;
  p.dp_salt = dp_salt; p.frames_per_sample = frames_per_sample > 0 ? frames_per_sample : 1;
  p.per_frame = per_frame; p.total4 = (long long)frames * per_frame / 4;
}

}

using namespace npvp;

#define LN_LAUNCH(kernel, C, ...)                                                                         \
  switch ((C) / 256) {                                                                                    \
    case 1: NPVP_LAUNCH(kernel<1>, __VA_ARGS__); break;  case 2: NPVP_LAUNCH(kernel<2>, __VA_ARGS__); break;   \
    case 3: NPVP_LAUNCH(kernel<3>, __VA_ARGS__); break;  default: NPVP_LAUNCH(kernel<4>, __VA_ARGS__); break;  \
  }

extern "C" int npvp_layernorm_fwd(const float* x, const float* w, const float* b, float* y, float* mean, float* rstd,
                                  long long rows, int C, float eps, int relu, float* amax, hipStream_t stream) {
  NPVP_CHECK_ARG(rows > 0, "layernorm: no rows");
  NPVP_CHECK_ARG(C % 256 == 0 && C >= 256 && C <= 1024, "layernorm: C must be 256, 512, 768 or 1024");
  const long long nb = (rows + 3) / 4;
  LN_LAUNCH(ln_fwd_kernel, C, dim3((unsigned)(nb > 4096 ? 4096 : nb)), dim3(256), 0, stream, x, w, b, y, mean, rstd, rows, eps, relu, amax);
  NPVP_CHECK_LAUNCH();
  return NPVP_OK;
}

static int ln_bwd_blocks(long long rows) {
  long long b = (rows + 3) / 4;
  return (int)(b > 512 ? 512 : b);
}

static Partials ln_partials(const void* ws, float* dw, float* db, long long rows, int C, int accumulate) {
  const int nb = ln_bwd_blocks(rows);
  return make_partials(ws, 0, nb, nb, 2 * C, dw, accumulate, db, C);
}

extern "C" long long npvp_layernorm_bwd_workspace_bytes(long long rows, int C) {
  return ln_partials(nullptr, nullptr, nullptr, rows, C, 0).bytes;
}

extern "C" int npvp_layernorm_bwd(const float* dy, const float* x, const float* w, const float* b, const float* mean,
                                  const float* rstd, float* dx, float* dw, float* db, long long rows, int C, int relu,
                                  const float* dres, int accumulate, float* amax, void* workspace, long long ws_bytes,
                                  hipStream_t stream) {
  NPVP_CHECK_ARG(rows > 0, "layernorm_bwd: no rows");
  NPVP_CHECK_ARG(C % 256 == 0 && C >= 256 && C <= 1024, "layernorm_bwd: C must be 256, 512, 768 or 1024");
  const Partials P = ln_partials(workspace, dw, db, rows, C, accumulate);
  NPVP_CHECK_ARG(workspace && ws_bytes >= P.bytes, "layernorm_bwd: workspace too small");
  LN_LAUNCH(ln_bwd_kernel, C, dim3(P.job.nb), dim3(256), 0, stream, dy, x, w, b, mean, rstd, dx, P.part(), rows, relu, dres, amax);
  NPVP_CHECK_LAUNCH();
  return finish_partials(P.job, accumulate, stream, "layernorm_bwd: reduce launch failed");
}

extern "C" int npvp_layernorm_bwd_reduce(const void* workspace, float* dw, float* db, long long rows, int C, int accumulate,
                                         hipStream_t stream) {
  NPVP_CHECK_ARG(workspace && dw && db && rows > 0, "layernorm_bwd_reduce: bad arguments");
  return finish_partials(ln_partials(workspace, dw, db, rows, C, accumulate).job, 0, stream, "layernorm_bwd_reduce: launch failed");
}

extern "C" int npvp_layernorm_bwd_reduce_job(const void* workspace, float* dw, float* db, long long rows, int C, int accumulate, void* job) {
  NPVP_CHECK_ARG(workspace && dw && db && rows > 0 && job, "layernorm_bwd_reduce_job: bad arguments");
  return put_job(job, ln_partials(workspace, dw, db, rows, C, accumulate).job);
}

extern "C" int npvp_sum_rows_multi(const void* jobs, int n, hipStream_t stream) {
  NPVP_CHECK_ARG(jobs && n > 0, "sum_rows_multi: no jobs");
  const SumRowsJob* J = (const SumRowsJob*)jobs;
  for (int at = 0; at < n; at += SRJ_MAX) {
    SumRowsBatch b;
    b.n = n - at < SRJ_MAX ? n - at : SRJ_MAX;
    int blocks = 0;
    for (int i = 0; i < b.n; ++i) {
      b.j[i] = J[at + i];
      NPVP_CHECK_ARG(b.j[i].in && b.j[i].out && b.j[i].nb > 0 && b.j[i].ncols > 0, "sum_rows_multi: bad job");
      b.cw[i] = plan_sum_rows(b.j[i]).cw;
      b.first[i] = blocks;
      blocks += (b.j[i].ncols + b.cw[i] - 1) / b.cw[i];
    }
    b.first[b.n] = blocks;
    NPVP_LAUNCH(sum_rows_multi_kernel, dim3(blocks), dim3(1024), 0, stream, b);
    NPVP_CHECK_LAUNCH();
  }
  return NPVP_OK;
}

extern "C" int npvp_layernorm_nchw_fwd(const float* x, const float* w, const float* b, float* out, float* mean, float* rstd,
                                       int frames, int P, int C, float eps, int relu, hipStream_t stream) {
// ... 71 lines not shown
  NPVP_CHECK_ARG(!dgamma || dyxh, "posfuse_bwd: this shape needs the dy*uhat scratch (dyxh) for dgamma");
  const long long total4 = (long long)frames * per_frame / 4;
  NPVP_LAUNCH(posfuse_bwd_apply_kernel, dim3(ew_blocks(total4, 256)), dim3(256), 0, stream, dy, x, add, gamma, mean,
                     rstd, (const float*)s1, (const float*)s2, du, dgamma ? dyxh : nullptr, T, per_frame, total4);
  NPVP_CHECK_LAUNCH();
  if (dbeta) { const int rc = npvp_reduce_mid_launch(dy, dbeta, 1, N, (long long)T * per_frame, 1.f, stream, accumulate); if (rc) return rc; }
  if (dgamma) { const int rc = npvp_reduce_mid_launch(dyxh, dgamma, 1, N, (long long)T * per_frame, 1.f, stream, accumulate); if (rc) return rc; }
  return NPVP_OK;
}

extern "C" int npvp_posfuse_instance_fwd(const float* x, const float* add, const float* beta, const float* gamma, float* y,
                                         float* mean, float* rstd, int N, int T, int P, int C, float eps, float* y_amax,
                                         hipStream_t stream) {
  NPVP_CHECK_ARG(N > 0 && T > 0 && P > 0 && P <= PFI_MAXP && C > 0, "posfuse_instance: bad shape (P <= 64)");
  NPVP_LAUNCH(posfuse_inst_fwd_kernel, dim3((C + 255) / 256, N * T), dim3(256), 0, stream, x, add, beta, gamma, y, mean,
                     rstd, T, P, C, eps, y_amax);
  NPVP_CHECK_LAUNCH();
  return NPVP_OK;
}

extern "C" int npvp_posfuse_instance_bwd(const float* dy, const float* x, const float* add, const float* gamma, const float* mean,
                                         const float* rstd, float* du, float* dyxh, int N, int T, int P, int C,
                                         hipStream_t stream) {
  NPVP_CHECK_ARG(N > 0 && T > 0 && P > 0 && P <= PFI_MAXP && C > 0, "posfuse_instance_bwd: bad shape (P <= 64)");
  NPVP_LAUNCH(posfuse_inst_bwd_kernel, dim3((C + 255) / 256, N * T), dim3(256), 0, stream, dy, x, add, gamma, mean, rstd,
                     du, dyxh, T, P, C);
  NPVP_CHECK_LAUNCH();
  return NPVP_OK;
}

extern "C" int npvp_frameln_act_fwd(const float* h, const float* mean, const float* rstd, const float* w, const float* b,
                                    const float* res, float* out, int frames, int per_frame, float drop_p,
                                    unsigned int salt, float dp_p, unsigned int dp_salt, int frames_per_sample,
                                    const unsigned long long* seed, float* amax, hipStream_t stream) {
  NPVP_CHECK_ARG(frames > 0 && per_frame % 4 == 0, "frameln_act: bad shape");
  NPVP_CHECK_ARG((drop_p == 0.f && dp_p == 0.f) || seed, "frameln_act: dropout needs a device seed");
  FlnParams p;
  fill_fln(p, h, mean, rstd, w, b, res, frames, per_frame, drop_p, salt, dp_p, dp_salt, frames_per_sample, seed);
  NPVP_LAUNCH(frameln_act_fwd_kernel, dim3(ew_blocks(p.total4, 256)), dim3(256), 0, stream, p, out, amax);
  NPVP_CHECK_LAUNCH();
  return NPVP_OK;
}

extern "C" int npvp_frameln_act_fwd_parts(const float* h, const float* part, int J, float nb, float eps, float* mean, float* rstd,
                                          const float* w, const float* b, const float* res, float* out, int frames,
                                          int per_frame, float drop_p, unsigned int salt, float dp_p, unsigned int dp_salt,
                                          int frames_per_sample, const unsigned long long* seed, float* amax, hipStream_t stream) {
  NPVP_CHECK_ARG(frames > 0 && per_frame % 4096 == 0 && part && J > 0 && nb > 0.f && mean && rstd, "frameln_act_fwd_parts: bad arguments");
  NPVP_CHECK_ARG((drop_p == 0.f && dp_p == 0.f) || seed, "frameln_act: dropout needs a device seed");
  NPVP_CHECK_ARG((long long)frames * (per_frame / 4096) < (1ll << 31), "frameln_act_fwd_parts: too many blocks");
  FlnParams p;
  fill_fln(p, h, nullptr, nullptr, w, b, res, frames, per_frame, drop_p, salt, dp_p, dp_salt, frames_per_sample, seed);
  NPVP_LAUNCH(frameln_act_fwd_parts_kernel, dim3((unsigned)((long long)frames * (per_frame / 4096))), dim3(256), 0, stream, p,
                     part, J, nb, eps, mean, rstd, out, amax);
  NPVP_CHECK_LAUNCH();
  return NPVP_OK;
}

static int fln_chunks(int frames) {
  if (frames >= 512) return 32;
  const int c = frames / 2 < 16 ? frames / 2 : 16;
  return c < 1 ? 1 : c;
}

static Partials fln_partials(const void* ws, float* dw, float* db, int frames, int per_frame, int accumulate) {
  return make_partials(ws, (long long)frames * 2 * FLN_PARTS, frames, fln_chunks(frames), 2 * per_frame, dw, accumulate, db, per_frame);
}

extern "C" long long npvp_frameln_act_bwd_workspace_bytes(int frames, int per_frame) {
  return fln_partials(nullptr, nullptr, nullptr, frames, per_frame, 0).bytes;
}

static int fln_bwd_fused(const FlnParams& p, const float* dout, const float* psum, int nparts, float* dh, const Partials& P, int frames,
                         int accumulate, float* amax, hipStream_t stream, const char* error) {
  NPVP_LAUNCH(frameln_act_bwd_fused_kernel, dim3((p.per_frame / 4 + 255) / 256, P.job.nb), dim3(256), 0, stream, p,
                     dout, psum, dh, P.part(), frames, P.per, nparts, amax);
  NPVP_CHECK_LAUNCH();
  return finish_partials(P.job, accumulate, stream, error);
}

extern "C" int npvp_frameln_act_bwd(const float* dout, const float* h, const float* mean, const float* rstd, const float* w,
                                    const float* b, float* dh, float* dw, float* db, int frames, int per_frame,
                                    float drop_p, unsigned int salt, float dp_p, unsigned int dp_salt,
                                    int frames_per_sample, const unsigned long long* seed, int accumulate, float* amax,
                                    void* workspace, long long ws_bytes, hipStream_t stream) {
  NPVP_CHECK_ARG(frames > 0 && per_frame % 4 == 0, "frameln_act_bwd: bad shape");
  const Partials P = fln_partials(workspace, dw, db, frames, per_frame, accumulate);
  NPVP_CHECK_ARG(workspace && ws_bytes >= P.bytes, "frameln_act_bwd: workspace too small");
  FlnParams p;
  fill_fln(p, h, mean, rstd, w, b, nullptr, frames, per_frame, drop_p, salt, dp_p, dp_salt, frames_per_sample, seed);
  NPVP_CHECK_ARG(per_frame % (4 * FLN_PARTS) == 0, "frameln_act_bwd: per_frame must be a multiple of 16");
  NPVP_LAUNCH(frameln_act_bwd_stats_kernel, dim3(frames, FLN_PARTS), dim3(512), 0, stream, p, dout, (float*)workspace);
  NPVP_CHECK_LAUNCH();
  return fln_bwd_fused(p, dout, (const float*)workspace, FLN_PARTS, dh, P, frames, accumulate, amax, stream, "frameln_act_bwd: reduce launch failed");
}

extern "C" int npvp_frameln_act_bwd_apply(const float* dout, const float* h, const float* mean, const float* rstd, const float* w,
                                          const float* b, const float* psum, int nparts, float* dh, float* dw, float* db,
                                          int frames, int per_frame, int accumulate, float* amax, void* workspace,
                                          long long ws_bytes, hipStream_t stream) {
  NPVP_CHECK_ARG(frames > 0 && per_frame % 4 == 0 && psum && nparts > 0, "frameln_act_bwd_apply: bad arguments");
  const Partials P = fln_partials(workspace, dw, db, frames, per_frame, accumulate);
  NPVP_CHECK_ARG(workspace && ws_bytes >= P.bytes, "frameln_act_bwd_apply: workspace too small");
  FlnParams p;
  fill_fln(p, h, mean, rstd, w, b, nullptr, frames, per_frame, 0.f, 0u, 0.f, 0u, 1, nullptr);
  return fln_bwd_fused(p, dout, psum, nparts, dh, P, frames, accumulate, amax, stream, "frameln_act_bwd_apply: reduce launch failed");
}

extern "C" int npvp_frameln_act_bwd_pgrad(const float* dout, const float* h, const float* mean, const float* rstd, const float* w,
                                          const float* b, float* psum, float* dw, float* db, int frames, int per_frame,
                                          float drop_p, unsigned int salt, float dp_p, unsigned int dp_salt, int frames_per_sample,
                                          const unsigned long long* seed, int accumulate, void* workspace, long long ws_bytes,
                                          hipStream_t stream) {
  NPVP_CHECK_ARG(frames > 0 && per_frame % 1024 == 0 && psum, "frameln_act_bwd_pgrad: per_frame must be a multiple of 1024");
  const Partials P = fln_partials(workspace, dw, db, frames, per_frame, accumulate);
  NPVP_CHECK_ARG(workspace && ws_bytes >= P.bytes, "frameln_act_bwd_pgrad: workspace too small");
  FlnParams p;
  fill_fln(p, h, mean, rstd, w, b, nullptr, frames, per_frame, drop_p, salt, dp_p, dp_salt, frames_per_sample, seed);
  NPVP_LAUNCH(frameln_act_bwd_pgrad_kernel, dim3(per_frame / 1024, P.job.nb), dim3(256), 0, stream, p, dout, psum,
                     P.part(), frames, P.per);
  NPVP_CHECK_LAUNCH();
  return finish_partials(P.job, accumulate, stream, "frameln_act_bwd_pgrad: reduce launch failed");
}

extern "C" int npvp_frameln_act_bwd_reduce_job(const void* workspace, float* dw, float* db, int frames, int per_frame, int accumulate,
                                               void* job) {
  NPVP_CHECK_ARG(workspace && dw && db && frames > 0 && job, "frameln_act_bwd_reduce_job: bad arguments");
  return put_job(job, fln_partials(workspace, dw, db, frames, per_frame, accumulate).job);
}

extern "C" int npvp_frameln_act_bwd_reduce(const void* workspace, float* dw, float* db, int frames, int per_frame,
                                           int accumulate, hipStream_t stream) {
  NPVP_CHECK_ARG(workspace && dw && db && frames > 0, "frameln_act_bwd_reduce: bad arguments");
  return finish_partials(fln_partials(workspace, dw, db, frames, per_frame, accumulate).job, 0, stream, "frameln_act_bwd_reduce: launch failed");
}
```

### npvp_amd/ops.py

```python
import ctypes
import os

import torch

from ._lib import lib, check
from . import sched as _S
from .sched import (_p, _ptr, _stream, _ws, AmaxSlot, GemmProbe, HbmProbe, ProbeEvent, probe_pair, AuxStream, StepContext, current, use, scoped,
                    remember, rng, GradSink, WgradStream, WgradChain, ReduceQueue, RangeGuard)


def amax_of(t, slot=None):
    if slot is not None:
        return slot
    for cand in (t, t._base):
        tag = getattr(cand, "_npvp_amax", None) if cand is not None else None
        if tag is not None and tag[1] == cand._version:
            return tag[0]
    s = AmaxSlot.new(t.device)
    t2 = t if t.dim() == 2 else t.reshape(-1, t.shape[-1])
    if t2.stride(1) != 1:
        t2 = t2.contiguous()
    check(lib().npvp_amax(_ptr(t2), t2.shape[0], t2.shape[1], t2.stride(0), _ptr(s), _stream()), "npvp_amax")
    t._npvp_amax = (s, t._version)
    return s
# ... 148 lines not shown
            ent.F, ent.D = ent.planes[0], ent.planes[1]
            cls._split(ent)
            store[key] = ent
            cls._dirty = True
        elif ent.version != w._version:
            cls._split(ent)
        if w._base is None and tuple(w.shape) == tuple(ent.w.shape):
            w.__dict__["_npvp_ent"] = (ent, w.data_ptr(), cls._gen)
        return (ent.F if want == "F" else ent.D), ent.amax

    @classmethod
    def _entries(cls):
        live = []
        for ref in cls._owners:
            owner = ref()
            if owner is None:
                continue
            live.append(ref)
            for ent in owner.__dict__.get("_npvp_planes", {}).values():
                yield ent
        cls._owners = live

    @classmethod
    def refresh_if_stale(cls):
        if any(ent.version != ent.w._version for ent in cls._entries()):
            cls.refresh_all()

    epoch = 0

    @classmethod
    def refresh_all(cls, owner=None):
        cls.epoch += 1
        if not cls.enabled:
            return
        if cls._dirty or cls._tables is None:
            owner = None
            groups = {}
            for ent in cls._entries():
                if ent.w.is_cuda:
                    groups.setdefault((ent.w.untyped_storage().data_ptr(), ent.fmt, ent.w.device), []).append(ent)
            cls._tables = []
            kept = {}
            for gkey, ents in groups.items():
                own_id, fmt, dev = gkey
                ids = tuple(id(e) for e in ents)
                old = cls._group_tensors.get(gkey)
                if old is not None and old[0] == ids and (fmt != 6 or all(e.amax_t is old[2] for e in ents)):
                    table, amax_t = old[1], old[2]
                else:
                    amax_t = None
                    if fmt == 6:
                        amax_t = torch.zeros(len(ents), AmaxSlot.FLOATS, dtype=torch.float32, device=dev)
                        for i, ent in enumerate(ents):
                            ent.amax_t = amax_t
                            ent.amax.ptr, ent.amax.chunk = amax_t.data_ptr() + AmaxSlot.BYTES * i, amax_t
                    rows = []
                    for ent in ents:
                        N, K = ent.w.shape
                        r = [ent.w.data_ptr(), ent.w.stride(0), N, K, ent.planes[0].data_ptr(), ent.planes[1].data_ptr()]
                        rows.append(r + [ent.amax.ptr, 0] if fmt == 6 else r)
                    table = torch.tensor(rows, dtype=torch.int64).to(dev)
                kept[gkey] = (ids, table, amax_t)
                cls._tables.append((fmt, table, amax_t, ents, own_id))
            cls._group_tensors = kept
            cls._dirty = False
        only = None if owner is None else owner.untyped_storage().data_ptr()
        for fmt, table, amax_t, ents, own_id in cls._tables:
            if only is not None and own_id != only:
                continue
            with torch.cuda.device(table.device):
                if fmt == 6:
                    check(lib().npvp_split_weights_f16(_p(table.data_ptr()), table.shape[0], _p(amax_t.data_ptr()),
                                                       amax_t.numel() * 4, _stream()), "npvp_split_weights_f16")
                else:
                    check(lib().npvp_split_weights_batched(_p(table.data_ptr()), table.shape[0], _stream()), "npvp_split_weights_batched")
            for ent in ents:
                ent.version = ent.w._version




def gemm(a_kc, b_kc, M, N, K, A, lda, B, ldb, out, bias=None, act=0, aux_in=None, aux_out=None, residual=None,
         drop=NO_DROP, alpha=1.0, colsum_a=None, b_pre=None, accumulate=False, rowstats=None, precision=None,
         replay=False, a_amax=None, b_amax=None, c_amax=None, a_drop=NO_DROP, range_flag=None):
    for t in (A, B, out, bias, aux_in, aux_out, residual, colsum_a):
        if t is not None and not (t.is_cuda and t.dtype is torch.float32):
            _chk(t)
    prec = GEMM_PRECISION if precision is None else precision
    planes = None
    if b_pre is not None:
        planes, b_amax = b_pre
    if prec == 6:
        kid = _gemm_kernel_id(a_kc, b_kc, M, N, K, 6, planes is not None)
        if kid == 5 or kid == 7:
            if a_amax is None:
                a_amax = amax_of(A)
        elif kid == 6:
            if a_amax is None:
                a_amax = amax_of(A)
            if b_amax is None:
                b_amax = amax_of(B)
        else:
            planes = None
    wsb = _gemm_ws_bytes(M, N, K)
    ws, wsn = (None, 0)
    if wsb > 0:
        ws, wsn = _ws(wsb, A.device)
    masked = drop.p > 0.0 or a_drop.p > 0.0
    seed = _S._cur.rng.seed_tensor(A.device) if masked else None
    if DropRecorder.sites is not None and not replay:
        DropRecorder.note(drop, "elem" if drop.mode == 0 else "group", M * N if drop.mode == 0 else drop.g2)
    probe = GemmProbe.armed
    if probe:
        kid = _gemm_kernel_id(a_kc, b_kc, M, N, K, prec, planes is not None)
        probe = GemmProbe.only is None or kid in GemmProbe.only
    if probe:
        e0, e1 = probe_pair()
    rc = lib().npvp_gemm_f32(
        a_kc, b_kc, M, N, K, A.data_ptr(), lda, B.data_ptr(), ldb, out.data_ptr(), out.stride(0),
        None if bias is None else bias.data_ptr(), act, None if aux_in is None else aux_in.data_ptr(),
        None if aux_out is None else aux_out.data_ptr(), None if residual is None else residual.data_ptr(),
        0 if residual is None else residual.stride(0), drop.p, drop.mode, drop.g1, drop.g2,
        None if seed is None else seed.data_ptr(), drop.salt, alpha, prec, None if colsum_a is None else colsum_a.data_ptr(),
        None if planes is None else planes.data_ptr(), 1 if accumulate else 0, None if rowstats is None else rowstats.data_ptr(),
        None if a_amax is None else a_amax.data_ptr(), None if b_amax is None else b_amax.data_ptr(),
        None if c_amax is None else c_amax.data_ptr(), None if range_flag is None else range_flag.data_ptr(),
        a_drop.p, a_drop.g1, a_drop.g2, a_drop.salt, None if ws is None else ws.data_ptr(), wsn, _stream())
    if rc:
        check(rc, "npvp_gemm_f32")
    if probe:
        e1.record()
        GemmProbe.records.append((e0, e1, 2.0 * M * N * K, 4.0 * (M * K + N * K + M * N), ((a_kc, b_kc), kid)))
    return out


_KID_CACHE, _WSB_CACHE = {}, {}


def _gemm_kernel_id(a_kc, b_kc, M, N, K, prec, has_planes):
    key = (a_kc, b_kc, M, N, K, prec, has_planes)
    v = _KID_CACHE.get(key)
    if v is None:
        v = _KID_CACHE[key] = lib().npvp_gemm_kernel_id(a_kc, b_kc, M, N, K, prec, int(has_planes))
    return v


def _gemm_ws_bytes(M, N, K):
    v = _WSB_CACHE.get((M, N, K))
    if v is None:
        v = _WSB_CACHE[(M, N, K)] = lib().npvp_gemm_workspace_bytes(M, N, K)
    return v


def _planes(w, want, R):
    return WeightPlanes.get(w, want) if R >= 256 else None


def _new_slot(dev, want=True):
    return AmaxSlot.new(dev) if (want and GEMM_PRECISION == 6) else None


def linear_fwd(x, w, b, act=0, aux_out=None, residual=None, drop=NO_DROP, rowstats=None, x_amax=None, y_amax=None):
    R, K = x.shape
    N = w.shape[0]
    y = torch.empty(R, N, dtype=torch.float32, device=x.device)
    return gemm(1, 1, R, N, K, x, x.stride(0), w, w.stride(0), y, bias=b, act=act, aux_out=aux_out, residual=residual,
                drop=drop, b_pre=_planes(w, "F", R), rowstats=rowstats, a_amax=x_amax, c_amax=y_amax)


def linear_frame_stats_supported(R, N):
    return GEMM_PRECISION in (4, 6) and R % 64 == 0 and N % 128 == 0


def linear_dgrad(dy, w, act=0, aux_in=None, drop=NO_DROP, residual=None, dy_amax=None, dx_amax=None, a_drop=NO_DROP, out=None,
                 accumulate=False):
    R, N = dy.shape
    K = w.shape[1]
    dx = torch.empty(R, K, dtype=torch.float32, device=dy.device) if out is None else out
    return gemm(1, 0, R, K, N, dy, dy.stride(0), w, w.stride(0), dx, act=act, aux_in=aux_in, drop=drop, residual=residual,
                b_pre=_planes(w, "D", R), replay=True, a_amax=dy_amax, c_amax=dx_amax, a_drop=a_drop, accumulate=accumulate)


def masked_grad(dy2, drop, w):
    if not drop.on:
        return dy2, NO_DROP
    R, N = dy2.shape
    K = w.shape[1]
    if (drop.mode == 1 and drop.g1 % 16 == 0 and drop.p < 0.5 and GEMM_PRECISION == 6 and R <= DROP_PATH_IN_GEMM_ROWS
            and _planes(w, "D", R) is not None and _gemm_kernel_id(1, 0, R, K, N, 6, True) in (5, 7)
            and _gemm_kernel_id(0, 0, N, K, R, 6, False) == 6):
        return dy2, drop
    return drop_apply(dy2, drop), NO_DROP


DROP_PATH_IN_GEMM_ROWS = 1 << 30


def linear_wgrad(dy, x, with_bias_grad=False, into=None, into_b=None, dy_amax=None, x_amax=None, a_drop=NO_DROP):
    R, N = dy.shape
    K = x.shape[1]
    acc = into is not None
    dw = into if acc else torch.empty(N, K, dtype=torch.float32, device=dy.device)
    db = (into_b if acc else torch.empty(N, dtype=torch.float32, device=dy.device)) if with_bias_grad else None
    prec = WGRAD_PRECISION if GEMM_PRECISION == 4 else None
    watch = GEMM_PRECISION == 6 and _gemm_kernel_id(0, 0, N, K, R, 6, False) == 6
    if watch and _S._cur.range_guard.fallback and not a_drop.on:
        prec, watch = 4, False
    if watch and _S._cur.range_guard.strict and not a_drop.on:
        flag = _S._cur.range_guard.flag(dy.device)
        tw = torch.empty(N, K, dtype=torch.float32, device=dy.device)
        tb = torch.empty(N, dtype=torch.float32, device=dy.device) if with_bias_grad else None
        gemm(0, 0, N, K, R, dy, dy.stride(0), x, x.stride(0), tw, colsum_a=tb, a_amax=dy_amax, b_amax=x_amax, range_flag=flag)
        if _S._cur.range_guard.poll(dy.device):
            _S._cur.range_guard.fallback = False
            gemm(0, 0, N, K, R, dy, dy.stride(0), x, x.stride(0), tw, colsum_a=tb, precision=4)
        if acc:
            dw.add_(tw)
            if tb is not None:
                db.add_(tb)
        else:
            dw, db = tw, tb
        return (dw, db) if with_bias_grad else dw
    flag = _S._cur.range_guard.flag(dy.device) if watch else None
    on_side = _S._cur.wgrad.in_flush
    if (watch and acc and prec is None and _S._cur.chain.enabled and _S._cur.chain.takes(N, K, R)
            and (on_side or (not _S._cur.wgrad.enabled and _S._cur.grad_sink.listener is None))
            and dy.stride(1) == 1 and x.stride(1) == 1 and dw.stride(1) == 1):
        _S._cur.chain.launch(dy, x, dw, db, amax_of(dy, dy_amax), amax_of(x, x_amax), a_drop, flag)
        if not on_side:
            _S._cur.reduce._arm()
        return (dw, db) if with_bias_grad else dw
    gemm(0, 0, N, K, R, dy, dy.stride(0), x, x.stride(0), dw, colsum_a=db, accumulate=acc, precision=prec, a_amax=dy_amax, b_amax=x_amax,
         a_drop=a_drop, range_flag=flag)
    return (dw, db) if with_bias_grad else dw


class FusedLinearBwd:
    enabled = True
    MAX_ROWS = 16384
    with_gradient_stream = False
    _ok = {}

    @classmethod
    def takes(cls, R, N, K):
        key = (R, N, K)
        v = cls._ok.get(key)
        if v is None:
            v = cls._ok[key] = bool(lib().npvp_linear_bwd_f16_takes(R, N, K)) and _S._cur.chain.takes(N, K, R)
        return v and R <= cls.MAX_ROWS


def linear_bwd(dy, x, w, b, sk, act=0, aux_in=None, drop=NO_DROP, residual=None, dy_amax=None, dx_amax=None, a_drop=NO_DROP):
    R, N = dy.shape
    K = w.shape[1]
    has_b = b is not None
    if (FusedLinearBwd.enabled and GEMM_PRECISION == 6 and sk and has_b == (sk[1] is not None) and FusedLinearBwd.takes(R, N, K)
            and (FusedLinearBwd.with_gradient_stream or not _S._cur.wgrad.enabled) and not _S._cur.range_guard.fallback and not _S._cur.range_guard.strict and dy.stride(1) == 1 and x.stride(1) == 1):
        pl = _planes(w, "D", R)
        gw = sk[0][0]
        if pl is not None and gw.stride(1) == 1:
            planes, w_amax = pl
            gb = sk[1][0] if has_b else None
            dev = dy.device
            dy_amax, x_amax = amax_of(dy, dy_amax), amax_of(x)
            dx = torch.empty(R, K, dtype=torch.float32, device=dev)
            ws, wsn = _ws(_S._cur.chain._wsb[(N, K, R)], dev)
            st = _stream()
            seed = _S._cur.rng.seed_tensor(dev) if (drop.on or a_drop.on) else None
            outs = (gw.data_ptr(),) if gb is None else (gw.data_ptr(), gb.data_ptr())
            chain = not _S._cur.wgrad.enabled
            if chain:
                job = ctypes.create_string_buffer(64)
                prev = _S._cur.chain._pending.pop(st, None)
                job_addr, prev_addr = ctypes.addressof(job), (ctypes.addressof(prev[0]) if prev is not None else None)
            else:
                job_addr, prev_addr = _S._cur.reduce.splitk_slot(outs), None
            probe = GemmProbe.armed and (GemmProbe.only is None or 8 in GemmProbe.only)
            if probe:
                e0, e1 = probe_pair()
            check(lib().npvp_linear_bwd_f16(R, N, K, dy.data_ptr(), dy.stride(0), dy_amax.data_ptr(), planes.data_ptr(), w_amax.data_ptr(),
                                            dx.data_ptr(), dx.stride(0), act, _ptr(aux_in), _ptr(residual),
                                            0 if residual is None else residual.stride(0), drop.p, drop.mode, drop.g1, drop.g2, drop.salt,
                                            _ptr(dx_amax), x.data_ptr(), x.stride(0), x_amax.data_ptr(), gw.data_ptr(), gw.stride(0),
                                            _ptr(gb), _ptr(_S._cur.range_guard.flag(dev)), a_drop.p, a_drop.g1, a_drop.g2, a_drop.salt, _ptr(seed),
                                            prev_addr, job_addr, ws.data_ptr(), wsn, st), "npvp_linear_bwd_f16")
            if probe:
                e1.record()
                GemmProbe.records.append((e0, e1, 4.0 * R * N * K, 4.0 * (2 * R * N + 2 * R * K + 2 * N * K), ((1, 0), 8)))
            if chain:
                if prev is not None and prev[4] is not None:
                    _S._cur.grad_sink.wrote(*prev[4])
                _S._cur.chain._pending[st] = (job, ws, gw, gb, sk)
                _S._cur.reduce._arm()
            else:
                _S._cur.reduce.splitk_added(outs, ws, sk)
            return dx, None, None
    dx = linear_dgrad(dy, w, act=act, aux_in=aux_in, drop=drop, residual=residual, dy_amax=dy_amax, dx_amax=dx_amax, a_drop=a_drop)
    gw, gb = _lin_grads(dy, x, w, b, sk, a_drop=a_drop)
    return dx, gw, gb


def colsum(x):
    R, N = x.shape
    L = lib()
    out = torch.empty(N, dtype=torch.float32, device=x.device)
    ws, wsn = _ws(L.npvp_colsum_workspace_bytes(R, N), x.device)
    check(L.npvp_colsum(_ptr(x), R, N, x.stride(0), _ptr(out), 0, _ptr(ws), wsn, _stream()), "npvp_colsum")
    return out


def drop_apply(x2d, drop):
    out = torch.empty_like(x2d)
    slot = _new_slot(x2d.device)
    check(lib().npvp_drop_apply(_ptr(x2d), _ptr(out), x2d.shape[0], x2d.shape[1], drop.p, drop.mode, drop.g1, drop.g2,
                                _ptr(_S._cur.rng.seed_tensor(x2d.device)), drop.salt, _ptr(slot), _stream()), "npvp_drop_apply")
    return tag_amax(out, slot)


def transpose(x):
    _chk(x)
    x = _c(x)
    B, R, C = x.shape
    out = torch.empty(B, C, R, dtype=torch.float32, device=x.device)
    check(lib().npvp_transpose(_ptr(x), _ptr(out), B, R, C, _stream()), "npvp_transpose")
    return out


def reduce_mid(x, scale=1.0, out=None, accumulate=False):
    _chk(x)
    x = _c(x)
    A, B, C = x.shape
    if out is None:
        out = torch.empty(A, C, dtype=torch.float32, device=x.device)
    check(lib().npvp_reduce_mid(_ptr(x), _ptr(out), A, B, C, scale, 1 if accumulate else 0, _stream()), "npvp_reduce_mid")
    return out


class ActSink:
    __slots__ = ("buf",)
    enabled = True

    def __init__(self):
        self.buf = None

    def target(self, shape, dev):
        if self.buf is None:
            self.buf = torch.empty(shape, dtype=torch.float32, device=dev)
            return self.buf, False
        if self.buf.numel() != torch.Size(shape).numel():
            raise RuntimeError(f"ActSink: a consumer contributes a gradient of shape {tuple(shape)} to a buffer of shape {tuple(self.buf.shape)}")
        return self.buf, True

    @staticmethod
    def of(t):
        return None if t is None else getattr(t, "_npvp_sink", None)


class _FanOut(torch.autograd.Function):
    @staticmethod
    def forward(ctx, t, sink):
        ctx.sink = sink
        ctx.set_materialize_grads(False)
        return t.view_as(t)

    @staticmethod
    def backward(ctx, g):
        buf, ctx.sink.buf = ctx.sink.buf, None
        if buf is None:
            return g, None
        if g is not None:
            buf.add_(g.reshape(buf.shape))
        return buf, None


def fan_out(t):
    if t is None or not (ActSink.enabled and t.is_cuda and t.requires_grad and torch.is_grad_enabled()):
        return t
    sink = ActSink()
    out = _FanOut.apply(t, sink)
    out._npvp_sink = sink
# ... 454 lines not shown
    slot = _new_slot(q.device)
    fn, what = (lib().npvp_attn_long_fwd, "npvp_attn_long_fwd") if _attn_long(cfg) else (lib().npvp_attn_fwd, "npvp_attn_fwd")
    check(fn(_ptr(q), q.stride(0), _ptr(k), k.stride(0), _ptr(v), v.stride(0), _ptr(o), o.stride(0),
             cfg.mode, cfg.dim0, cfg.P, cfg.W, cfg.ws, cfg.Tq, cfg.Tk, cfg.heads, hd, cfg.mask_mode,
             cfg.drop.p, _ptr(seed), cfg.drop.salt, _ptr(slot), _stream()), what)
    tag_amax(o, slot)


def _attn_bwd(q, k, v, go, dq, dk, dv, cfg, packed=None):
    hd = go.shape[1] // cfg.heads
    seed = _S._cur.rng.seed_tensor(q.device) if cfg.drop.on else None
    sq = _new_slot(q.device)
    sk = sq if packed is not None else _new_slot(q.device)
    sv = _new_slot(q.device)
    args = (_ptr(q), q.stride(0), _ptr(k), k.stride(0), _ptr(v), v.stride(0), _ptr(go), go.stride(0),
            _ptr(dq), dq.stride(0), _ptr(dk), dk.stride(0), _ptr(dv), dv.stride(0), cfg.mode, cfg.dim0,
            cfg.P, cfg.W, cfg.ws, cfg.Tq, cfg.Tk, cfg.heads, hd, cfg.mask_mode, cfg.drop.p, _ptr(seed),
            cfg.drop.salt, _ptr(sq), _ptr(sk), _ptr(sv))
    if _attn_long(cfg):
        ws, wsn = _ws(lib().npvp_attn_long_bwd_workspace_bytes(cfg.mode, cfg.dim0, cfg.P, cfg.W, cfg.ws, cfg.Tq, cfg.Tk, cfg.heads),
                      q.device)
        check(lib().npvp_attn_long_bwd(*args, _ptr(ws), wsn, _stream()), "npvp_attn_long_bwd")
    else:
        check(lib().npvp_attn_bwd(*args, _stream()), "npvp_attn_bwd")
    if packed is not None:
        tag_amax(packed, sq)
    else:
        tag_amax(dq, sq); tag_amax(dk, sk)
    tag_amax(dv, sv)


class _AttnPacked(torch.autograd.Function):

    @staticmethod
    def forward(ctx, qk, v, cfg):
        remember(ctx)
        _chk(qk, v)
        C = v.shape[1]
        o = torch.empty_like(v)
        _attn_fwd(qk[:, :C], qk[:, C:], v, o, cfg)
        ctx.save_for_backward(qk, v)
        ctx.cfg = cfg
        return o

    @scoped
    def backward(ctx, go):
        qk, v = ctx.saved_tensors
        C = v.shape[1]
        go = _c(go)
        dqk, dv = torch.empty_like(qk), torch.empty_like(v)
        _attn_bwd(qk[:, :C], qk[:, C:], v, go, dqk[:, :C], dqk[:, C:], dv, ctx.cfg, packed=dqk)
        return dqk, dv, None


class _Attn(torch.autograd.Function):

    @staticmethod
    def forward(ctx, q, k, v, cfg):
        remember(ctx)
        _chk(q, k, v)
        o = torch.empty_like(q)
        _attn_fwd(q, k, v, o, cfg)
        ctx.save_for_backward(q, k, v)
        ctx.cfg = cfg
        return o

    @scoped
    def backward(ctx, go):
        q, k, v = ctx.saved_tensors
        go = _c(go)
        dq, dk, dv = torch.empty_like(q), torch.empty_like(k), torch.empty_like(v)
        _attn_bwd(q, k, v, go, dq, dk, dv, ctx.cfg)
        return dq, dk, dv, None


def attn_packed(qk, v, cfg):
    return _AttnPacked.apply(qk, v, cfg)


def attn(q, k, v, cfg):
    return _Attn.apply(q, k, v, cfg)


def _fln_bwd(dout, h, mean, rstd, w, b, frames, PF, d, dp, T, sk, psum=None, nparts=0, want_amax=True):
    L = lib()
    dev = h.device
    dh = torch.empty_like(h)
    slot = _new_slot(dev, want_amax)
    tag_amax(dh, slot)
    dw, db = (sk[0][0], sk[1][0]) if sk else (torch.empty_like(w), torch.empty_like(b))
    ws, wsn = _ws(L.npvp_frameln_act_bwd_workspace_bytes(frames, PF), dev)
    mode = _sink_mode(sk)
    if psum is None:
        seed = _S._cur.rng.seed_tensor(dev) if (d.on or dp.on) else None
        check(L.npvp_frameln_act_bwd(_ptr(dout), _ptr(h), _ptr(mean), _ptr(rstd), _ptr(w), _ptr(b), _ptr(dh), _ptr(dw), _ptr(db),
                                     frames, PF, d.p, d.salt, dp.p, dp.salt, T, _ptr(seed), mode, _ptr(slot), _ptr(ws), wsn,
                                     _stream()), "npvp_frameln_act_bwd")
    else:
        pe = HbmProbe.begin()
        check(L.npvp_frameln_act_bwd_apply(_ptr(dout), _ptr(h), _ptr(mean), _ptr(rstd), _ptr(w), _ptr(b), _ptr(psum), nparts,
                                           _ptr(dh), _ptr(dw), _ptr(db), frames, PF, mode, _ptr(slot), _ptr(ws), wsn, _stream()),
              "npvp_frameln_act_bwd_apply")
        HbmProbe.end(pe, "npvp::frameln_act_bwd_fused_kernel", 4.0 * 3 * frames * PF)
    if sk:
        _reduce_partials(sk, ws, dw, db, L.npvp_frameln_act_bwd_reduce, L.npvp_frameln_act_bwd_reduce_job, "npvp_frameln_act_bwd_reduce",
                         (frames, PF, 1), True)
        return dh, None, None
    return dh, dw, db


def _fln_pgrad(dout, h, mean, rstd, w, b, frames, PF, d, sk):
    L = lib()
    dev = h.device
    psum = torch.empty(frames * (PF // 1024) * 2, dtype=torch.float32, device=dev)
    dw, db = (sk[0][0], sk[1][0]) if sk else (torch.empty_like(w), torch.empty_like(b))
    ws, wsn = _ws(L.npvp_frameln_act_bwd_workspace_bytes(frames, PF), dev)
    seed = _S._cur.rng.seed_tensor(dev) if d.on else None
    check(L.npvp_frameln_act_bwd_pgrad(_ptr(dout), _ptr(h), mean, rstd, _ptr(w), _ptr(b), _ptr(psum), _ptr(dw), _ptr(db),
                                       frames, PF, d.p, d.salt, 0.0, 0, 1, _ptr(seed), _sink_mode(sk), _ptr(ws), wsn, _stream()),
          "npvp_frameln_act_bwd_pgrad")
    if sk:
        _reduce_partials(sk, ws, dw, db, L.npvp_frameln_act_bwd_reduce, L.npvp_frameln_act_bwd_reduce_job, "npvp_frameln_act_bwd_reduce",
                         (frames, PF, 1), True)
        return psum, None, None
    return psum, dw, db


class _FrameLnAct(torch.autograd.Function):

    @staticmethod
    def forward(ctx, h, w_cl, b_cl, res, frames, p_drop, p_dp, frames_per_sample, mean=None, rstd=None):
        remember(ctx)
        _chk(h, w_cl, b_cl, res)
        h = _c(h)
        PF = h.numel() // frames
        w_cl, b_cl = _c(w_cl), _c(b_cl)
        res_c = None if res is None else _c(res)
        L = lib()
        if mean is None:
            mean = torch.empty(frames, dtype=torch.float32, device=h.device)
            rstd = torch.empty_like(mean)
            check(L.npvp_frame_stats(_ptr(h), _p(0), _ptr(mean), _ptr(rstd), frames, 1, PF, 1e-5, _stream()), "npvp_frame_stats")
        d, dp = Drop(p_drop), Drop(p_dp, 1)
        DropRecorder.note(d, "elem", h.numel())
        DropRecorder.note(dp, "group", frames // max(1, frames_per_sample))
        out = torch.empty_like(h)
        seed = _S._cur.rng.seed_tensor(h.device) if (d.on or dp.on) else None
        slot = _new_slot(h.device)
        check(L.npvp_frameln_act_fwd(_ptr(h), _ptr(mean), _ptr(rstd), _ptr(w_cl), _ptr(b_cl), _ptr(res_c), _ptr(out), frames,
                                     PF, d.p, d.salt, dp.p, dp.salt, frames_per_sample, _ptr(seed), _ptr(slot), _stream()),
              "npvp_frameln_act_fwd")
        tag_amax(out, slot)
        ctx.save_for_backward(h, mean, rstd, w_cl, b_cl)
        ctx.cfg = (frames, PF, d, dp, frames_per_sample, res is not None)
        ctx.sink = _ln_sink(w_cl, b_cl)
        return out

    @scoped
    def backward(ctx, dout):
        h, mean, rstd, w_cl, b_cl = ctx.saved_tensors
        frames, PF, d, dp, fps, has_res = ctx.cfg
        dout = _c(dout)
        dh, dw, db = _fln_bwd(dout, h, mean, rstd, w_cl, b_cl, frames, PF, d, dp, fps, ctx.sink)
        return dh, dw, db, (dout if has_res else None), None, None, None, None, None, None


def frameln_act(h, w_cl, b_cl, res, frames, p_drop=0.0, p_dp=0.0, frames_per_sample=1, stats=None):
    mean, rstd = stats if stats is not None else (None, None)
    return _FrameLnAct.apply(h, w_cl, b_cl, res, frames, p_drop, p_dp, frames_per_sample, mean, rstd)


class _DwConv(torch.autograd.Function):

    @staticmethod
    def forward(ctx, a, wtb, frames, H, W, want_stats):
        remember(ctx)
        _chk(a, wtb)
        a, wtb = _c(a), _c(wtb)
        Ch = wtb.shape[1]
        out = torch.empty_like(a)
        ctx.save_for_backward(a, wtb)
        ctx.cfg = (frames, H, W, Ch)
        if want_stats:
            mean = torch.empty(frames, dtype=torch.float32, device=a.device)
            rstd = torch.empty_like(mean)
            ws, wsn = _ws(frames * (Ch // 1024) * 8, a.device)
            check(lib().npvp_dwconv3x3_stats(_ptr(a), _ptr(wtb), _row(wtb, 9), _ptr(out), _ptr(mean), _ptr(rstd), frames, H, W,
                                             Ch, 1e-5, _ptr(ws), wsn, _stream()), "npvp_dwconv3x3_stats")
            ctx.mark_non_differentiable(mean, rstd)
            ctx.set_materialize_grads(False)
            return out, mean, rstd
        check(lib().npvp_dwconv3x3(_ptr(a), _ptr(wtb), _row(wtb, 9), _ptr(out), frames, H, W, Ch, 0, _stream()),
              "npvp_dwconv3x3")
        return out

    @scoped
    def backward(ctx, dout, *_unused):
        a, wtb = ctx.saved_tensors
        frames, H, W, Ch = ctx.cfg
        dout = _c(dout)
        L = lib()
        da = torch.empty_like(a)
        check(L.npvp_dwconv3x3(_ptr(dout), _ptr(wtb), _p(0), _ptr(da), frames, H, W, Ch, 1, _stream()), "npvp_dwconv3x3(bwd)")
        dwtb = torch.empty_like(wtb)
        ws, wsn = _ws(L.npvp_dwconv3x3_wgrad_workspace_bytes(frames, Ch), a.device)
        check(L.npvp_dwconv3x3_wgrad(_ptr(a), _ptr(dout), _ptr(dwtb), frames, H, W, Ch, _ptr(ws), wsn, _stream()),
              "npvp_dwconv3x3_wgrad")
        return da, dwtb, None, None, None, None


def dwconv3x3(a, wtb, frames, H, W, want_stats=False):
    return _DwConv.apply(a, wtb, frames, H, W, bool(want_stats))


class _MlpDwbn(torch.autograd.Function):

    @staticmethod
    def forward(ctx, x, res, w1, b1, n1w, n1b, dww, dwb, n2w, n2b, w2, b2, n3w, n3b, frames, T, p_drop, p_dp):
        remember(ctx)
        _chk(x, res, w1, b1, w2, b2)
        L = lib()
        R, C = x.shape
        hid, Co = w1.shape[0], w2.shape[0]
        dev, f32 = x.device, torch.float32
        st = _stream()
        PFh, PFo = 64 * hid, 64 * Co
        h1 = torch.empty(R, hid, dtype=f32, device=dev)
        part = torch.empty(frames * (hid // 64) * 2, dtype=f32, device=dev)
        gemm(1, 1, R, hid, C, x, x.stride(0), w1, w1.stride(0), h1, bias=b1, b_pre=_planes(w1, "F", R),
             rowstats=part)
        stats = torch.empty(6, frames, dtype=f32, device=dev)
        key = (WeightPlanes.epoch, dww._version, dwb._version, dww.data_ptr(), dwb.data_ptr())
        hit = dww.__dict__.get("_npvp_wtb")
        if hit is not None and hit[0] == key:
            wtb = hit[1]
        else:
            wtb = torch.empty(10, hid, dtype=f32, device=dev)
            check(L.npvp_dwtb_build(_ptr(_c(dww)), _ptr(dwb), _ptr(wtb), hid, st), "npvp_dwtb_build")
            dww.__dict__["_npvp_wtb"] = (key, wtb)
        h2 = torch.empty(R, hid, dtype=f32, device=dev)
        part2 = torch.empty(frames * (hid // 512) * 2, dtype=f32, device=dev)
        check(L.npvp_mlpdw_mid_fwd_parts(_ptr(h1), _ptr(part), hid // 64, 4096.0, _row(stats, 0), _row(stats, 1), _ptr(n1w), _ptr(n1b),
                                         _ptr(wtb), _row(wtb, 9), _ptr(h2), _ptr(part2), frames, 8, 8, hid, 1e-5, st),
              "npvp_mlpdw_mid_fwd_parts")
        d2, d3, dp = Drop(p_drop), Drop(p_drop), Drop(p_dp, 1)
        DropRecorder.note(d2, "elem", R * hid)
        seed = _S._cur.rng.seed_tensor(dev) if (d2.on or dp.on) else None
        a2 = torch.empty(R, hid, dtype=f32, device=dev)
        a2_slot = _new_slot(dev)
        check(L.npvp_frameln_act_fwd_parts(_ptr(h2), _ptr(part2), hid // 512, 32768.0, 1e-5, _row(stats, 2), _row(stats, 3), _ptr(n2w),
                                           _ptr(n2b), None, _ptr(a2), frames, PFh, d2.p, d2.salt, 0.0, 0, 1, _ptr(seed), _ptr(a2_slot),
                                           st), "npvp_frameln_act_fwd_parts")
        tag_amax(a2, a2_slot)
        h3 = torch.empty(R, Co, dtype=f32, device=dev)
        part3 = torch.empty(frames * (Co // 64) * 2, dtype=f32, device=dev)
        gemm(1, 1, R, Co, hid, a2, hid, w2, w2.stride(0), h3, bias=b2, b_pre=_planes(w2, "F", R),
             rowstats=part3)
        DropRecorder.note(d3, "elem", R * Co)
        DropRecorder.note(dp, "group", frames // max(1, T))
        out = torch.empty(R, Co, dtype=f32, device=dev)
        check(L.npvp_frameln_act_fwd_parts(_ptr(h3), _ptr(part3), Co // 64, 4096.0, 1e-5, _row(stats, 4), _row(stats, 5), _ptr(n3w),
                                           _ptr(n3b), _ptr(res), _ptr(out), frames, PFo, d3.p, d3.salt, dp.p, dp.salt, T, _ptr(seed),
                                           None, st), "npvp_frameln_act_fwd_parts")
        ctx.save_for_backward(x, h1, h2, a2, h3, stats, wtb, w1, w2, n1w, n1b, n2w, n2b, n3w, n3b)
        ctx.cfg = (frames, T, d2, d3, dp, res is not None, b1 is not None, b2 is not None)
        ctx.sinks = (_wb_sink(w1, b1), _wb_sink(w2, b2), _ln_sink(n1w, n1b), _ln_sink(n2w, n2b), _ln_sink(n3w, n3b))
        sd = _wb_sink(dww, dwb) if (dww.is_contiguous() and dwb is not None) else None
        ctx.sink_dw = sd if (sd and sd[1] is not None) else None
        return out

    @scoped
    def backward(ctx, dout):
        x, h1, h2, a2, h3, stats, wtb, w1, w2, n1w, n1b, n2w, n2b, n3w, n3b = ctx.saved_tensors
        frames, T, d2, d3, dp, has_res, has_b1, has_b2 = ctx.cfg
        s_fc1, s_fc2, s_n1, s_n2, s_n3 = ctx.sinks
        L = lib()
        R, hid = h1.shape
        Co = h3.shape[1]
        dev = x.device
        dout = _c(dout)
        dh3, gn3w, gn3b = _fln_bwd(dout, h3, stats[4], stats[5], n3w, n3b, frames, 64 * Co, d3, dp, T, s_n3)
        da2, gw2, gb2 = linear_bwd(dh3, a2, w2, True if has_b2 else None, s_fc2)
        fuse_n2 = MID_BWD_N2 and hid // 16 <= 256
        if fuse_n2:
            psum2, gn2w, gn2b = _fln_pgrad(da2, h2, _row(stats, 2), _row(stats, 3), n2w, n2b, frames, 64 * hid, d2, s_n2)
        else:
            dh2, gn2w, gn2b = _fln_bwd(da2, h2, stats[2], stats[3], n2w, n2b, frames, 64 * hid, d2, NO_DROP, 1, s_n2,
                                          want_amax=False)
            del da2
        da1 = torch.empty_like(h1)
        dwtb = torch.empty(10, hid, dtype=torch.float32, device=dev)
        nparts = hid // 256
        psum = torch.empty(frames * nparts * 2, dtype=torch.float32, device=dev)
        ws, wsn = _ws(L.npvp_mlpdw_mid_bwd_workspace_bytes(frames, hid), dev)
        sk_dw = ctx.sink_dw if ctx.needs_input_grad[6] and ctx.needs_input_grad[7] else None
        wmode = 2 if sk_dw else 0
        if fuse_n2:
            seed = _S._cur.rng.seed_tensor(dev) if d2.on else None
            pe = HbmProbe.begin()
            check(L.npvp_mlpdw_mid_bwd_n2(_ptr(da2), _ptr(h2), _row(stats, 2), _row(stats, 3), _ptr(n2w), _ptr(n2b), _ptr(psum2),
                                          hid // 16, d2.p, d2.salt, _ptr(seed), _ptr(h1), _row(stats, 0), _row(stats, 1), _ptr(n1w),
                                          _ptr(n1b), _ptr(wtb), _ptr(da1), _ptr(dwtb), _ptr(psum), frames, 8, 8, hid, wmode, _ptr(ws), wsn,
                                          _stream()), "npvp_mlpdw_mid_bwd_n2")
            HbmProbe.end(pe, "npvp::mlpdw_mid_bwd_kernel<1, true>", 4.0 * 4 * frames * 64 * hid)
            del da2, psum2
        else:
            check(L.npvp_mlpdw_mid_bwd(_ptr(dh2), _ptr(h1), _row(stats, 0), _row(stats, 1), _ptr(n1w), _ptr(n1b), _ptr(wtb), _ptr(da1),
                                       _ptr(dwtb), _ptr(psum), frames, 8, 8, hid, wmode, _ptr(ws), wsn, _stream()), "npvp_mlpdw_mid_bwd")
            del dh2
        if sk_dw:
            _reduce_partials(sk_dw, ws, sk_dw[0][0], sk_dw[1][0], L.npvp_mlpdw_mid_bwd_reduce_into, L.npvp_mlpdw_mid_bwd_reduce_job,
                             "npvp_mlpdw_mid_bwd_reduce_into", (frames, hid), False)
            gdww = gdwb = None
        else:
            gdww = torch.empty(hid, 1, 3, 3, dtype=torch.float32, device=dev)
            check(L.npvp_transpose(_ptr(dwtb), _ptr(gdww), 1, 9, hid, _stream()), "npvp_transpose")
            gdwb = dwtb[9]
        dh1, gn1w, gn1b = _fln_bwd(da1, h1, stats[0], stats[1], n1w, n1b, frames, 64 * hid, NO_DROP, NO_DROP, 1, s_n1,
                                      psum=psum, nparts=nparts)
        del da1
        dx, gw1, gb1 = linear_bwd(dh1, x, w1, True if has_b1 else None, s_fc1)
        return (dx, dout if has_res else None, gw1, gb1, gn1w, gn1b, gdww, gdwb, gn2w, gn2b, gw2, gb2, gn3w, gn3b,
                None, None, None, None)


MID_BWD_N2 = True


def mlpdwbn_fused_supported(R, C, hid, Co, H, W):
    return (GEMM_PRECISION in (4, 6) and H == 8 and W == 8 and R % 64 == 0 and hid % 512 == 0 and Co % 128 == 0 and hid % 128 == 0
            and C % 32 == 0)


def mlpdwbn(x, res, w1, b1, n1w, n1b, dww, dwb, n2w, n2b, w2, b2, n3w, n3b, frames, T, p_drop, p_dp):
    return _MlpDwbn.apply(x, res, w1, b1, n1w, n1b, dww, dwb, n2w, n2b, w2, b2, n3w, n3b, frames, T, p_drop, p_dp)


def _raw_ln_fwd(x2, w, b, eps, relu=0):
    rows, C = x2.shape
    y = torch.empty_like(x2)
    st = torch.empty(2, rows, dtype=torch.float32, device=x2.device)
    slot = _new_slot(x2.device)
    check(lib().npvp_layernorm_fwd(_ptr(x2), _ptr(w), _ptr(b), _ptr(y), _row(st, 0), _row(st, 1), rows, C, eps, relu, _ptr(slot),
                                   _stream()), "npvp_layernorm_fwd")
    return tag_amax(y, slot), st


def _raw_ln_bwd(dy2, x2, w, b, st, dres, sk, relu=0, probe=False):
    L = lib()
    rows, C = x2.shape
    dx = torch.empty_like(x2)
    dw, db = (sk[0][0], sk[1][0]) if sk else (torch.empty_like(w), torch.empty_like(b))
    ws, wsn = _ws(L.npvp_layernorm_bwd_workspace_bytes(rows, C), x2.device)
    slot = _new_slot(x2.device)
    pe = HbmProbe.begin() if probe else None
    check(L.npvp_layernorm_bwd(_ptr(dy2), _ptr(x2), _ptr(w), _ptr(b), _row(st, 0), _row(st, 1), _ptr(dx), _ptr(dw), _ptr(db), rows, C,
                               relu, _ptr(dres), _sink_mode(sk), _ptr(slot), _ptr(ws), wsn, _stream()), "npvp_layernorm_bwd")
    HbmProbe.end(pe, "npvp::ln_bwd_kernel<2>", 4.0 * (3 + (dres is not None)) * rows * C)
    tag_amax(dx, slot)
    if sk:
        _reduce_partials(sk, ws, dw, db, L.npvp_layernorm_bwd_reduce, L.npvp_layernorm_bwd_reduce_job, "npvp_layernorm_bwd_reduce",
                         (rows, C, 1), True)
        return dx, None, None
    return dx, dw, db


def _raw_posfuse_fwd(x, add, beta, gamma, N, T):
    PF = x.numel() // (N * T)
    y = torch.empty_like(x)
    st = torch.empty(2, N * T, dtype=torch.float32, device=x.device)
    slot = _new_slot(x.device)
    check(lib().npvp_posfuse_fwd(_ptr(x), _ptr(add), _ptr(beta), _ptr(gamma), _ptr(y), _row(st, 0), _row(st, 1), N, T, PF, 1e-5,
                                 _ptr(slot), _stream()), "npvp_posfuse_fwd")
    return tag_amax(y, slot), st


LN_POSFUSE_ONE_KERNEL = True


def _raw_ln_posfuse_fwd(x2, lw, lb, eps, add, beta, gamma, N, T):
    rows, C = x2.shape
    if not (LN_POSFUSE_ONE_KERNEL and C == 512 and rows == N * T * 64):
        x1, lst = _raw_ln_fwd(x2, lw, lb, eps)
        fused, pst = _raw_posfuse_fwd(x1, add, beta, gamma, N, T)
        return x1, lst, fused, pst
    x1, fused = torch.empty_like(x2), torch.empty_like(x2)
    lst = torch.empty(2, rows, dtype=torch.float32, device=x2.device)
    pst = torch.empty(2, N * T, dtype=torch.float32, device=x2.device)
    s1, s2 = _new_slot(x2.device), _new_slot(x2.device)
    check(lib().npvp_ln_posfuse_fwd(_ptr(x2), _ptr(lw), _ptr(lb), eps, _ptr(x1), _row(lst, 0), _row(lst, 1), _ptr(add), _ptr(beta),
                                    _ptr(gamma), _ptr(fused), _row(pst, 0), _row(pst, 1), N, T, 64, C, 1e-5, _ptr(s1), _ptr(s2),
                                    _stream()), "npvp_ln_posfuse_fwd")
    return tag_amax(x1, s1), lst, tag_amax(fused, s2), pst


def _raw_posfuse_bwd(dy, x, add, beta_shape, gamma, st, N, T, want_add, sinks=(None, None, None)):
    PF = x.numel() // (N * T)
    du, dbeta, dgamma = _posfuse_bwd_call(dy, x, add, gamma, st, N, T, PF, beta_shape, True, gamma is not None,
                                          sinks[0], sinks[1])
    dadd = None
    if add is not None and want_add:
        if sinks[2] is not None:
            buf, acc = sinks[2].target(add.shape, x.device)
            reduce_mid(du.view(N, T, PF), out=buf.view(N, PF), accumulate=acc)
        else:
            dadd = reduce_mid(du.view(N, T, PF)).view(add.shape)
    return du, dadd, dbeta, dgamma


# ... 445 lines not shown
```

Measured before the change: 8520.

## Skip backward GEMM and norm work for samples dropped by drop-path

Adds a skip mode that works out, from the drop-path RNG, which samples (frame groups) were dropped. It then bypasses their backward work. In the fp16 GEMM kernel, a block whose rows all belong to dropped groups skips the MFMA main loop and runs only the epilogue on zeros. The frame-LN backward kernels (pgrad, apply, fused) write zeros for dropped frames and skip their math. Savings depend on the drop-path probability and on tile alignment with sample boundaries. The change adds per-block RNG checks and a new argument to several kernel interfaces.

```diff
diff --git a/include/npvp_hip.h b/include/npvp_hip.h
--- a/include/npvp_hip.h
+++ b/include/npvp_hip.h
@@ -29,6 +29,13 @@
                   const void* b_pre, int accumulate, float* rowstats, const float* a_amax, const float* b_amax,
                   float* c_amax, unsigned int* range_flag, float adrop_p, int adrop_g1, int adrop_g2, unsigned int adrop_salt,
                   void* workspace, long long ws_bytes, npvp_stream_t stream);
+int npvp_gemm_f32_skip(int a_kc, int b_kc, int M, int N, int K, const float* A, long long lda, const float* B, long long ldb,
+                       float* C, long long ldc, const float* bias, int act, const float* aux_in, float* aux_out,
+                       const float* residual, long long ldr, float drop_p, int drop_mode, int drop_g1, int drop_g2,
+                       const unsigned long long* seed, unsigned int salt, float alpha, int precision, float* colsum_a,
+                       const void* b_pre, int accumulate, float* rowstats, const float* a_amax, const float* b_amax,
+                       float* c_amax, unsigned int* range_flag, float adrop_p, int adrop_g1, int adrop_g2, unsigned int adrop_salt,
+                       int adrop_skip, void* workspace, long long ws_bytes, npvp_stream_t stream);
 int npvp_frame_stats_finalize(const float* part, int parts_per_frame, float values_per_part, float* mean, float* rstd,
                               int frames, float eps, npvp_stream_t stream);
 int npvp_split_weight(const float* w, long long ld, int N, int K, void* F, void* D, npvp_stream_t stream);
@@ -102,6 +109,7 @@
 int npvp_frameln_act_bwd(const float* dout, const float* h, const float* mean, const float* rstd, const float* w,
                          const float* b, float* dh, float* dw, float* db, int frames, int per_frame, float drop_p,
                          unsigned int salt, float dp_p, unsigned int dp_salt, int frames_per_sample,
+                         float skip_p, unsigned int skip_salt, int skip_fps,
                          const unsigned long long* seed, int accumulate ,
                          float* dh_amax, void* workspace, long long ws_bytes, npvp_stream_t stream);
 int npvp_frameln_act_bwd_reduce(const void* workspace, float* dw, float* db, int frames, int per_frame, int accumulate,
@@ -134,12 +142,13 @@
 int npvp_frameln_act_bwd_pgrad(const float* dout, const float* h, const float* mean, const float* rstd, const float* w,
                                const float* b, float* psum, float* dw, float* db, int frames, int per_frame, float drop_p,
                                unsigned int salt, float dp_p, unsigned int dp_salt, int frames_per_sample,
+                               float skip_p, unsigned int skip_salt, int skip_fps,
                                const unsigned long long* seed, int accumulate, void* workspace, long long ws_bytes,
                                npvp_stream_t stream);
 int npvp_frameln_act_bwd_apply(const float* dout, const float* h, const float* mean, const float* rstd, const float* w,
                                const float* b, const float* psum, int nparts, float* dh, float* dw, float* db, int frames,
-                               int per_frame, int accumulate, float* dh_amax, void* workspace, long long ws_bytes,
-                               npvp_stream_t stream);
+                               int per_frame, float skip_p, unsigned int skip_salt, int skip_fps, const unsigned long long* seed,
+                               int accumulate, float* dh_amax, void* workspace, long long ws_bytes, npvp_stream_t stream);
 
 int npvp_im2col3x3(const float* in, float* out, int frames, int H, int W, int C, int col2im, npvp_stream_t stream);
 long long npvp_dwconv3x3_wgrad_workspace_bytes(int frames, int Ch);
diff --git a/npvp_amd/_lib.py b/npvp_amd/_lib.py
--- a/npvp_amd/_lib.py
+++ b/npvp_amd/_lib.py
@@ -30,6 +30,9 @@
     "npvp_gemm_f32": (c_int, [c_int, c_int, c_int, c_int, c_int, c_p, c_ll, c_p, c_ll, c_p, c_ll, c_p, c_int, c_p, c_p,
                               c_p, c_ll, c_f, c_int, c_int, c_int, c_p, c_u, c_f, c_int, c_p, c_p, c_int, c_p, c_p, c_p, c_p, c_p,
                               c_f, c_int, c_int, c_u, c_p, c_ll, c_p]),
+    "npvp_gemm_f32_skip": (c_int, [c_int, c_int, c_int, c_int, c_int, c_p, c_ll, c_p, c_ll, c_p, c_ll, c_p, c_int, c_p, c_p,
+                                   c_p, c_ll, c_f, c_int, c_int, c_int, c_p, c_u, c_f, c_int, c_p, c_p, c_int, c_p, c_p, c_p, c_p, c_p,
+                                   c_f, c_int, c_int, c_u, c_int, c_p, c_ll, c_p]),
     "npvp_amax": (c_int, [c_p, c_ll, c_ll, c_ll, c_p, c_p]),
     "npvp_wgrad_f16_chainable": (c_int, [c_int, c_int, c_int]),
     "npvp_wgrad_f16_chain_workspace_bytes": (c_ll, [c_int, c_int, c_int]),
@@ -66,7 +69,7 @@
     "npvp_frameln_act_fwd": (c_int, [c_p, c_p, c_p, c_p, c_p, c_p, c_p, c_int, c_int, c_f, c_u, c_f, c_u, c_int, c_p, c_p, c_p]),
     "npvp_frameln_act_bwd_workspace_bytes": (c_ll, [c_int, c_int]),
     "npvp_frameln_act_bwd": (c_int, [c_p, c_p, c_p, c_p, c_p, c_p, c_p, c_p, c_p, c_int, c_int, c_f, c_u, c_f, c_u, c_int,
-                                     c_p, c_int, c_p, c_p, c_ll, c_p]),
+                                     c_f, c_u, c_int, c_p, c_int, c_p, c_p, c_ll, c_p]),
     "npvp_dwconv3x3": (c_int, [c_p, c_p, c_p, c_p, c_int, c_int, c_int, c_int, c_int, c_p]),
     "npvp_dwconv3x3_stats": (c_int, [c_p, c_p, c_p, c_p, c_p, c_p, c_int, c_int, c_int, c_int, c_f, c_p, c_ll, c_p]),
     "npvp_mlpdw_mid_fwd": (c_int, [c_p, c_p, c_p, c_p, c_p, c_p, c_p, c_p, c_p, c_p, c_int, c_int, c_int, c_int, c_f, c_p, c_ll, c_p]),
@@ -80,8 +83,9 @@
     "npvp_mlpdw_mid_bwd_n2": (c_int, [c_p, c_p, c_p, c_p, c_p, c_p, c_p, c_int, c_f, c_u, c_p, c_p, c_p, c_p, c_p, c_p, c_p, c_p, c_p,
                                       c_p, c_int, c_int, c_int, c_int, c_int, c_p, c_ll, c_p]),
     "npvp_frameln_act_bwd_pgrad": (c_int, [c_p, c_p, c_p, c_p, c_p, c_p, c_p, c_p, c_p, c_int, c_int, c_f, c_u, c_f, c_u, c_int,
-                                           c_p, c_int, c_p, c_ll, c_p]),
-    "npvp_frameln_act_bwd_apply": (c_int, [c_p, c_p, c_p, c_p, c_p, c_p, c_p, c_int, c_p, c_p, c_p, c_int, c_int, c_int, c_p, c_p, c_ll, c_p]),
+                                           c_f, c_u, c_int, c_p, c_int, c_p, c_ll, c_p]),
+    "npvp_frameln_act_bwd_apply": (c_int, [c_p, c_p, c_p, c_p, c_p, c_p, c_p, c_int, c_p, c_p, c_p, c_int, c_int, c_f, c_u, c_int, c_p,
+                                           c_int, c_p, c_p, c_ll, c_p]),
     "npvp_im2col3x3": (c_int, [c_p, c_p, c_int, c_int, c_int, c_int, c_int, c_p]),
     "npvp_dwconv3x3_wgrad_workspace_bytes": (c_ll, [c_int, c_int]),
     "npvp_dwconv3x3_wgrad": (c_int, [c_p, c_p, c_p, c_int, c_int, c_int, c_int, c_p, c_ll, c_p]),
diff --git a/npvp_amd/csrc/gemm.h b/npvp_amd/csrc/gemm.h
--- a/npvp_amd/csrc/gemm.h
+++ b/npvp_amd/csrc/gemm.h
@@ -26,6 +26,7 @@
   int act;
   DropSpec drop;
   DropSpec adrop;
+  int askip;
   int tiles_m, tiles_n;
   int splits;
   float alpha;
diff --git a/npvp_amd/csrc/gemm.hip b/npvp_amd/csrc/gemm.hip
--- a/npvp_amd/csrc/gemm.hip
+++ b/npvp_amd/csrc/gemm.hip
@@ -519,14 +519,16 @@
   return finish_partials(make_partials(p.colsum, 0, p.splits, p.splits, p.M, colsum_a, p.accum).job, 0, stream, "gemm: column-sum reduce launch failed");
 }
 
-extern "C" int npvp_gemm_f32(int a_kc, int b_kc, int M, int N, int K, const float* A, long long lda, const float* B,
-                             long long ldb, float* C, long long ldc, const float* bias, int act, const float* aux_in,
-                             float* aux_out, const float* residual, long long ldr, float drop_p, int drop_mode,
-                             int drop_g1, int drop_g2, const unsigned long long* seed, unsigned int salt, float alpha,
-                             int precision, float* colsum_a, const void* b_pre, int accumulate, float* rowstats,
-                             const float* a_amax, const float* b_amax, float* c_amax, unsigned int* range_flag,
-                             float adrop_p, int adrop_g1, int adrop_g2, unsigned int adrop_salt,
-                             void* workspace, long long ws_bytes, hipStream_t stream) {
+extern "C" int npvp_gemm_f32_skip(int a_kc, int b_kc, int M, int N, int K, const float* A, long long lda, const float* B,
+                                  long long ldb, float* C, long long ldc, const float* bias, int act, const float* aux_in,
+                                  float* aux_out, const float* residual, long long ldr, float drop_p, int drop_mode,
+                                  int drop_g1, int drop_g2, const unsigned long long* seed, unsigned int salt, float alpha,
+                                  int precision, float* colsum_a, const void* b_pre, int accumulate, float* rowstats,
+                                  const float* a_amax, const float* b_amax, float* c_amax, unsigned int* range_flag,
+                                  float adrop_p, int adrop_g1, int adrop_g2, unsigned int adrop_salt, int adrop_skip,
+                                  void* workspace, long long ws_bytes, hipStream_t stream) {
+  NPVP_CHECK_ARG(adrop_skip >= 0 && adrop_skip <= 3, "gemm: adrop_skip must be 0 .. 3 (bit 0: skip dropped work, bit 1: skip-only spec)");
+  NPVP_CHECK_ARG(adrop_skip == 0 || a_kc, "gemm: adrop_skip is for forward / dgrad launches (a_kc = 1)");
   NPVP_CHECK_ARG(M > 0 && N > 0 && K > 0, "gemm: empty problem");
   NPVP_CHECK_ARG(precision == 0 || precision == 4 || precision == 5 || precision == 6,
                  "gemm: precision must be 0 (exact fp32-input MFMA), 4 (three-term bf16 split, 6 MFMAs per product: "
@@ -564,6 +566,8 @@
   p.seed = seed; p.lda = lda; p.ldb = ldb; p.ldr = ldr; p.M = M; p.N = N; p.act = act;
   p.drop = make_drop_spec(drop_p, salt, drop_mode, drop_g1, drop_g2);
   p.adrop = make_drop_spec(adrop_p, adrop_salt, 1, adrop_g1, adrop_g2);
+  if (adrop_skip & 2) p.adrop.inv_keep = 1.f;
+  p.askip = (adrop_p > 0.f && (adrop_skip & 1)) ? 1 : 0;
   p.alpha = alpha;
   p.rowstats = rowstats;
   p.a_amax = a_amax; p.b_amax = b_amax; p.c_amax = c_amax; p.range_flag = range_flag;
@@ -602,3 +606,16 @@
   NPVP_CHECK_LAUNCH();
   return plan.splits > 1 ? finish_splitk(p, C, ldc, colsum_a, stream) : NPVP_OK;
 }
+
+extern "C" int npvp_gemm_f32(int a_kc, int b_kc, int M, int N, int K, const float* A, long long lda, const float* B,
+                             long long ldb, float* C, long long ldc, const float* bias, int act, const float* aux_in,
+                             float* aux_out, const float* residual, long long ldr, float drop_p, int drop_mode,
+                             int drop_g1, int drop_g2, const unsigned long long* seed, unsigned int salt, float alpha,
+                             int precision, float* colsum_a, const void* b_pre, int accumulate, float* rowstats,
+                             const float* a_amax, const float* b_amax, float* c_amax, unsigned int* range_flag,
+                             float adrop_p, int adrop_g1, int adrop_g2, unsigned int adrop_salt,
+                             void* workspace, long long ws_bytes, hipStream_t stream) {
+  return npvp_gemm_f32_skip(a_kc, b_kc, M, N, K, A, lda, B, ldb, C, ldc, bias, act, aux_in, aux_out, residual, ldr, drop_p, drop_mode,
+                            drop_g1, drop_g2, seed, salt, alpha, precision, colsum_a, b_pre, accumulate, rowstats, a_amax, b_amax, c_amax,
+                            range_flag, adrop_p, adrop_g1, adrop_g2, adrop_salt, 0, workspace, ws_bytes, stream);
+}
diff --git a/npvp_amd/csrc/gemm_f16.hip b/npvp_amd/csrc/gemm_f16.hip
--- a/npvp_amd/csrc/gemm_f16.hip
+++ b/npvp_amd/csrc/gemm_f16.hip
@@ -129,6 +129,33 @@
   const float zrow = 1.f;
   float rf0 = zrow, rf1 = zrow;
   const f32x16 zero16 = {0.f, 0.f, 0.f, 0.f, 0.f, 0.f, 0.f, 0.f, 0.f, 0.f, 0.f, 0.f, 0.f, 0.f, 0.f, 0.f};
+  if constexpr (!ROWSTATS) {
+    bool bypass = false;
+    if (p.askip && p.adrop.thresh) {
+      const unsigned long long aseed = *p.seed;
+      const unsigned int q_lo = div_by_magic((unsigned int)m0, p.adrop.m1, p.adrop.s1);
+      const unsigned int q_hi = div_by_magic((unsigned int)(min(m0 + BM, p.M) - 1), p.adrop.m1, p.adrop.s1);
+      bypass = true;
+      for (unsigned int q1 = q_lo; q1 <= q_hi; ++q1) {
+        const unsigned int grp = q1 - div_by_magic(q1, p.adrop.m2, p.adrop.s2) * (unsigned int)p.adrop.g2;
+        bypass = bypass && rng_u32(aseed, p.adrop.salt, (uint64_t)grp) < p.adrop.thresh;
+      }
+    }
+    if (bypass) {
+      const int row_base = m0 + wm * TM * 32, col_base = n0 + wn * TN * 32;
+      float cmax = 0.f;
+      float* scr = reinterpret_cast<float*>(lds) + 4 + wave * EPI_FLOATS;
+      const unsigned long long seed = (p.seed && p.drop.thresh) ? *p.seed : 0ull;
+      static_for<0, TM>([&](auto i) __attribute__((always_inline)) {
+        const float4 rowsc = epilogue_row_scales(p, seed, row_base + i * 32, lane);
+        static_for<0, TN>([&](auto j) __attribute__((always_inline)) {
+          epilogue_tile(p, zero16, row_base + i * 32, col_base + j * 32, lane, scr, 0, seed, cmax, rowsc, p.alpha);
+        });
+      });
+      amax_slot_commit_block(p.c_amax, cmax, reinterpret_cast<float*>(lds), cpeek);
+      return;
+    }
+  }
   auto run_tile = [&]() __attribute__((always_inline)) {
   NPVP_H_BLOAD(lds, 0)
   NPVP_H_ALOAD(ea0, ea1, 0)
diff --git a/npvp_amd/csrc/norm.hip b/npvp_amd/csrc/norm.hip
--- a/npvp_amd/csrc/norm.hip
+++ b/npvp_amd/csrc/norm.hip
@@ -553,11 +553,19 @@
   unsigned int drop_thresh; float drop_inv_keep; unsigned int salt;
   unsigned int dp_thresh; float dp_inv_keep; unsigned int dp_salt; int frames_per_sample;
   int per_frame; long long total4;
+  unsigned int skip_thresh; unsigned int skip_salt; int skip_fps;
 };
 
 __device__ __forceinline__ float fln_frame_scale(const FlnParams& p, unsigned long long seed, long long f) {
   if (!p.dp_thresh) return 1.f;
   return drop_scale(seed, p.dp_salt, (unsigned long long)((unsigned int)f / (unsigned int)p.frames_per_sample), p.dp_thresh, p.dp_inv_keep);
+}
+__device__ __forceinline__ bool fln_frame_skipped(const FlnParams& p, unsigned long long seed, long long f) {
+  if (!p.skip_thresh) return false;
+  return rng_u32(seed, p.skip_salt, (unsigned long long)((unsigned int)f / (unsigned int)p.skip_fps)) < p.skip_thresh;
+}
+__device__ __forceinline__ unsigned long long fln_seed(const FlnParams& p) {
+  return (p.seed && (p.drop_thresh || p.dp_thresh || p.skip_thresh)) ? *p.seed : 0ull;
 }
 __device__ __forceinline__ float fln_scale(const FlnParams& p, unsigned long long seed, float frame_scale, long long gidx) {
   if (!p.drop_thresh) return frame_scale;
@@ -626,7 +634,11 @@
                                                                     float* __restrict__ psum) {
   __shared__ float red[8];
   const long long f = blockIdx.x;
-  const unsigned long long seed = (p.seed && (p.drop_thresh || p.dp_thresh)) ? *p.seed : 0ull;
+  const unsigned long long seed = fln_seed(p);
+  if (fln_frame_skipped(p, seed, f)) {
+    if (threadIdx.x == 0) { psum[(f * FLN_PARTS + blockIdx.y) * 2] = 0.f; psum[(f * FLN_PARTS + blockIdx.y) * 2 + 1] = 0.f; }
+    return;
+  }
   const float mu = p.mean[f], rs = p.rstd[f];
   const float fsc = fln_frame_scale(p, seed, f);
   float s1 = 0.f, s2 = 0.f;
@@ -655,13 +667,17 @@
   const unsigned int peek = amax_peek_block(amax);
   float am = 0.f;
   if (e >= p.per_frame) { amax_slot_commit_block(amax, am, ared, peek); return; }
-  const unsigned long long seed = (p.seed && (p.drop_thresh || p.dp_thresh)) ? *p.seed : 0ull;
+  const unsigned long long seed = fln_seed(p);
   const float4 ww = ld4(p.w + e), bb = ld4(p.b + e);
   float4 aw = make_float4(0.f, 0.f, 0.f, 0.f), ab = make_float4(0.f, 0.f, 0.f, 0.f);
   const int f0 = blockIdx.y * frames_per_chunk;
   const int f1 = min(frames, f0 + frames_per_chunk);
   for (long long f = f0; f < f1; ++f) {
     const long long g0 = f * p.per_frame + e;
+    if (fln_frame_skipped(p, seed, f)) {
+      st4(dh + g0, make_float4(0.f, 0.f, 0.f, 0.f));
+      continue;
+    }
     const float mu = p.mean[f], rs = p.rstd[f];
     const float fsc = fln_frame_scale(p, seed, f);
     float a1 = 0.f, a2 = 0.f;
@@ -693,13 +709,17 @@
   __shared__ float red[4];
   const int e = (blockIdx.x * blockDim.x + threadIdx.x) * 4;
   const int nblk = gridDim.x;
-  const unsigned long long seed = (p.seed && (p.drop_thresh || p.dp_thresh)) ? *p.seed : 0ull;
+  const unsigned long long seed = fln_seed(p);
   const float4 ww = ld4(p.w + e), bb = ld4(p.b + e);
   float4 aw = make_float4(0.f, 0.f, 0.f, 0.f), ab = make_float4(0.f, 0.f, 0.f, 0.f);
   const int f0 = blockIdx.y * frames_per_chunk;
   const int f1 = min(frames, f0 + frames_per_chunk);
   for (long long f = f0; f < f1; ++f) {
     const long long g0 = f * p.per_frame + e;
+    if (fln_frame_skipped(p, seed, f)) {
+      if (threadIdx.x == 0) { psum[(f * nblk + blockIdx.x) * 2] = 0.f; psum[(f * nblk + blockIdx.x) * 2 + 1] = 0.f; }
+      continue;
+    }
     const float mu = p.mean[f], rs = p.rstd[f];
     const float fsc = fln_frame_scale(p, seed, f);
     const float4 v = ld4(p.h + g0), d = ld4(dout + g0);
@@ -786,6 +806,12 @@
   p.dp_inv_keep = dp_p > 0.f ? 1.f / (1.f - dp_p) : 1.f;
   p.dp_salt = dp_salt; p.frames_per_sample = frames_per_sample > 0 ? frames_per_sample : 1;
   p.per_frame = per_frame; p.total4 = (long long)frames * per_frame / 4;
+  p.skip_thresh = 0u; p.skip_salt = 0u; p.skip_fps = 1;
+}
+
+static void fill_fln_skip(FlnParams& p, float skip_p, unsigned int skip_salt, int skip_fps) {
+  p.skip_thresh = skip_p > 0.f ? drop_threshold(skip_p) : 0u;
+  p.skip_salt = skip_salt; p.skip_fps = skip_fps > 0 ? skip_fps : 1;
 }
 
 }
@@ -1023,13 +1049,16 @@
 extern "C" int npvp_frameln_act_bwd(const float* dout, const float* h, const float* mean, const float* rstd, const float* w,
                                     const float* b, float* dh, float* dw, float* db, int frames, int per_frame,
                                     float drop_p, unsigned int salt, float dp_p, unsigned int dp_salt,
-                                    int frames_per_sample, const unsigned long long* seed, int accumulate, float* amax,
+                                    int frames_per_sample, float skip_p, unsigned int skip_salt, int skip_fps,
+                                    const unsigned long long* seed, int accumulate, float* amax,
                                     void* workspace, long long ws_bytes, hipStream_t stream) {
   NPVP_CHECK_ARG(frames > 0 && per_frame % 4 == 0, "frameln_act_bwd: bad shape");
+  NPVP_CHECK_ARG(skip_p >= 0.f && skip_p < 1.f && (skip_p == 0.f || seed), "frameln_act_bwd: bad skip arguments");
   const Partials P = fln_partials(workspace, dw, db, frames, per_frame, accumulate);
   NPVP_CHECK_ARG(workspace && ws_bytes >= P.bytes, "frameln_act_bwd: workspace too small");
   FlnParams p;
   fill_fln(p, h, mean, rstd, w, b, nullptr, frames, per_frame, drop_p, salt, dp_p, dp_salt, frames_per_sample, seed);
+  fill_fln_skip(p, skip_p, skip_salt, skip_fps);
   NPVP_CHECK_ARG(per_frame % (4 * FLN_PARTS) == 0, "frameln_act_bwd: per_frame must be a multiple of 16");
   NPVP_LAUNCH(frameln_act_bwd_stats_kernel, dim3(frames, FLN_PARTS), dim3(512), 0, stream, p, dout, (float*)workspace);
   NPVP_CHECK_LAUNCH();
@@ -1038,26 +1067,32 @@
 
 extern "C" int npvp_frameln_act_bwd_apply(const float* dout, const float* h, const float* mean, const float* rstd, const float* w,
                                           const float* b, const float* psum, int nparts, float* dh, float* dw, float* db,
-                                          int frames, int per_frame, int accumulate, float* amax, void* workspace,
+                                          int frames, int per_frame, float skip_p, unsigned int skip_salt, int skip_fps,
+                                          const unsigned long long* seed, int accumulate, float* amax, void* workspace,
                                           long long ws_bytes, hipStream_t stream) {
   NPVP_CHECK_ARG(frames > 0 && per_frame % 4 == 0 && psum && nparts > 0, "frameln_act_bwd_apply: bad arguments");
+  NPVP_CHECK_ARG(skip_p >= 0.f && skip_p < 1.f && (skip_p == 0.f || seed), "frameln_act_bwd_apply: bad skip arguments");
   const Partials P = fln_partials(workspace, dw, db, frames, per_frame, accumulate);
   NPVP_CHECK_ARG(workspace && ws_bytes >= P.bytes, "frameln_act_bwd_apply: workspace too small");
   FlnParams p;
-  fill_fln(p, h, mean, rstd, w, b, nullptr, frames, per_frame, 0.f, 0u, 0.f, 0u, 1, nullptr);
+  fill_fln(p, h, mean, rstd, w, b, nullptr, frames, per_frame, 0.f, 0u, 0.f, 0u, 1, seed);
+  fill_fln_skip(p, skip_p, skip_salt, skip_fps);
   return fln_bwd_fused(p, dout, psum, nparts, dh, P, frames, accumulate, amax, stream, "frameln_act_bwd_apply: reduce launch failed");
 }
 
 extern "C" int npvp_frameln_act_bwd_pgrad(const float* dout, const float* h, const float* mean, const float* rstd, const float* w,
                                           const float* b, float* psum, float* dw, float* db, int frames, int per_frame,
                                           float drop_p, unsigned int salt, float dp_p, unsigned int dp_salt, int frames_per_sample,
+                                          float skip_p, unsigned int skip_salt, int skip_fps,
                                           const unsigned long long* seed, int accumulate, void* workspace, long long ws_bytes,
                                           hipStream_t stream) {
   NPVP_CHECK_ARG(frames > 0 && per_frame % 1024 == 0 && psum, "frameln_act_bwd_pgrad: per_frame must be a multiple of 1024");
+  NPVP_CHECK_ARG(skip_p >= 0.f && skip_p < 1.f && (skip_p == 0.f || seed), "frameln_act_bwd_pgrad: bad skip arguments");
   const Partials P = fln_partials(workspace, dw, db, frames, per_frame, accumulate);
   NPVP_CHECK_ARG(workspace && ws_bytes >= P.bytes, "frameln_act_bwd_pgrad: workspace too small");
   FlnParams p;
   fill_fln(p, h, mean, rstd, w, b, nullptr, frames, per_frame, drop_p, salt, dp_p, dp_salt, frames_per_sample, seed);
+  fill_fln_skip(p, skip_p, skip_salt, skip_fps);
   NPVP_LAUNCH(frameln_act_bwd_pgrad_kernel, dim3(per_frame / 1024, P.job.nb), dim3(256), 0, stream, p, dout, psum,
                      P.part(), frames, P.per);
   NPVP_CHECK_LAUNCH();
diff --git a/npvp_amd/ops.py b/npvp_amd/ops.py
--- a/npvp_amd/ops.py
+++ b/npvp_amd/ops.py
@@ -254,7 +254,7 @@
 
 def gemm(a_kc, b_kc, M, N, K, A, lda, B, ldb, out, bias=None, act=0, aux_in=None, aux_out=None, residual=None,
          drop=NO_DROP, alpha=1.0, colsum_a=None, b_pre=None, accumulate=False, rowstats=None, precision=None,
-         replay=False, a_amax=None, b_amax=None, c_amax=None, a_drop=NO_DROP, range_flag=None):
+         replay=False, a_amax=None, b_amax=None, c_amax=None, a_drop=NO_DROP, range_flag=None, a_skip=NO_DROP):
     for t in (A, B, out, bias, aux_in, aux_out, residual, colsum_a):
         if t is not None and not (t.is_cuda and t.dtype is torch.float32):
             _chk(t)
@@ -262,8 +262,11 @@
     planes = None
     if b_pre is not None:
         planes, b_amax = b_pre
+    askip = 0
     if prec == 6:
         kid = _gemm_kernel_id(a_kc, b_kc, M, N, K, 6, planes is not None)
+        if kid == 5 or kid == 7:
+            a_drop, askip = _a_mask(a_drop, a_skip)
         if kid == 5 or kid == 7:
             if a_amax is None:
                 a_amax = amax_of(A)
@@ -288,7 +291,7 @@
         probe = GemmProbe.only is None or kid in GemmProbe.only
     if probe:
         e0, e1 = probe_pair()
-    rc = lib().npvp_gemm_f32(
+    rc = lib().npvp_gemm_f32_skip(
         a_kc, b_kc, M, N, K, A.data_ptr(), lda, B.data_ptr(), ldb, out.data_ptr(), out.stride(0),
         None if bias is None else bias.data_ptr(), act, None if aux_in is None else aux_in.data_ptr(),
         None if aux_out is None else aux_out.data_ptr(), None if residual is None else residual.data_ptr(),
@@ -297,13 +300,21 @@
         None if planes is None else planes.data_ptr(), 1 if accumulate else 0, None if rowstats is None else rowstats.data_ptr(),
         None if a_amax is None else a_amax.data_ptr(), None if b_amax is None else b_amax.data_ptr(),
         None if c_amax is None else c_amax.data_ptr(), None if range_flag is None else range_flag.data_ptr(),
-        a_drop.p, a_drop.g1, a_drop.g2, a_drop.salt, None if ws is None else ws.data_ptr(), wsn, _stream())
+        a_drop.p, a_drop.g1, a_drop.g2, a_drop.salt, askip, None if ws is None else ws.data_ptr(), wsn, _stream())
     if rc:
-        check(rc, "npvp_gemm_f32")
+        check(rc, "npvp_gemm_f32_skip")
     if probe:
         e1.record()
         GemmProbe.records.append((e0, e1, 2.0 * M * N * K, 4.0 * (M * K + N * K + M * N), ((a_kc, b_kc), kid)))
     return out
+
+
+def _a_mask(a_drop, a_skip):
+    if a_drop.p > 0.0:
+        return a_drop, (1 if DROP_PATH_SKIP else 0)
+    if a_skip.p > 0.0 and DROP_PATH_SKIP and a_skip.mode == 1 and a_skip.p < 0.5:
+        return a_skip, 3
+    return a_drop, 0
 
 
 _KID_CACHE, _WSB_CACHE = {}, {}
@@ -345,12 +356,13 @@
 
 
 def linear_dgrad(dy, w, act=0, aux_in=None, drop=NO_DROP, residual=None, dy_amax=None, dx_amax=None, a_drop=NO_DROP, out=None,
-                 accumulate=False):
+                 accumulate=False, a_skip=NO_DROP):
     R, N = dy.shape
     K = w.shape[1]
     dx = torch.empty(R, K, dtype=torch.float32, device=dy.device) if out is None else out
     return gemm(1, 0, R, K, N, dy, dy.stride(0), w, w.stride(0), dx, act=act, aux_in=aux_in, drop=drop, residual=residual,
-                b_pre=_planes(w, "D", R), replay=True, a_amax=dy_amax, c_amax=dx_amax, a_drop=a_drop, accumulate=accumulate)
+                b_pre=_planes(w, "D", R), replay=True, a_amax=dy_amax, c_amax=dx_amax, a_drop=a_drop, accumulate=accumulate,
+                a_skip=a_skip)
 
 
 def masked_grad(dy2, drop, w):
@@ -422,7 +434,8 @@
         return v and R <= cls.MAX_ROWS
 
 
-def linear_bwd(dy, x, w, b, sk, act=0, aux_in=None, drop=NO_DROP, residual=None, dy_amax=None, dx_amax=None, a_drop=NO_DROP):
+def linear_bwd(dy, x, w, b, sk, act=0, aux_in=None, drop=NO_DROP, residual=None, dy_amax=None, dx_amax=None, a_drop=NO_DROP,
+               a_skip=NO_DROP):
     R, N = dy.shape
     K = w.shape[1]
     has_b = b is not None
@@ -467,7 +480,8 @@
             else:
                 _S._cur.reduce.splitk_added(outs, ws, sk)
             return dx, None, None
-    dx = linear_dgrad(dy, w, act=act, aux_in=aux_in, drop=drop, residual=residual, dy_amax=dy_amax, dx_amax=dx_amax, a_drop=a_drop)
+    dx = linear_dgrad(dy, w, act=act, aux_in=aux_in, drop=drop, residual=residual, dy_amax=dy_amax, dx_amax=dx_amax, a_drop=a_drop,
+                      a_skip=a_skip)
     gw, gb = _lin_grads(dy, x, w, b, sk, a_drop=a_drop)
     return dx, gw, gb
 
@@ -1088,7 +1102,14 @@
     return _Attn.apply(q, k, v, cfg)
 
 
-def _fln_bwd(dout, h, mean, rstd, w, b, frames, PF, d, dp, T, sk, psum=None, nparts=0, want_amax=True):
+def _skip_site(dp, T):
+    return (dp.p, dp.salt, T) if (DROP_PATH_SKIP and dp.on) else (0.0, 0, 1)
+
+
+def _fln_bwd(dout, h, mean, rstd, w, b, frames, PF, d, dp, T, sk, psum=None, nparts=0, want_amax=True, skip=NO_DROP):
+    if dp.on:
+        skip = dp
+    sp, ss, sf = _skip_site(skip, T)
     L = lib()
     dev = h.device
     dh = torch.empty_like(h)
@@ -1098,15 +1119,16 @@
     ws, wsn = _ws(L.npvp_frameln_act_bwd_workspace_bytes(frames, PF), dev)
     mode = _sink_mode(sk)
     if psum is None:
-        seed = _S._cur.rng.seed_tensor(dev) if (d.on or dp.on) else None
+        seed = _S._cur.rng.seed_tensor(dev) if (d.on or dp.on or sp > 0) else None
         check(L.npvp_frameln_act_bwd(_ptr(dout), _ptr(h), _ptr(mean), _ptr(rstd), _ptr(w), _ptr(b), _ptr(dh), _ptr(dw), _ptr(db),
-                                     frames, PF, d.p, d.salt, dp.p, dp.salt, T, _ptr(seed), mode, _ptr(slot), _ptr(ws), wsn,
-                                     _stream()), "npvp_frameln_act_bwd")
+                                     frames, PF, d.p, d.salt, dp.p, dp.salt, T, sp, ss, sf, _ptr(seed), mode, _ptr(slot),
+                                     _ptr(ws), wsn, _stream()), "npvp_frameln_act_bwd")
     else:
         pe = HbmProbe.begin()
+        seed = _S._cur.rng.seed_tensor(dev) if sp > 0 else None
         check(L.npvp_frameln_act_bwd_apply(_ptr(dout), _ptr(h), _ptr(mean), _ptr(rstd), _ptr(w), _ptr(b), _ptr(psum), nparts,
-                                           _ptr(dh), _ptr(dw), _ptr(db), frames, PF, mode, _ptr(slot), _ptr(ws), wsn, _stream()),
-              "npvp_frameln_act_bwd_apply")
+                                           _ptr(dh), _ptr(dw), _ptr(db), frames, PF, sp, ss, sf, _ptr(seed), mode, _ptr(slot), _ptr(ws),
+                                           wsn, _stream()), "npvp_frameln_act_bwd_apply")
         HbmProbe.end(pe, "npvp::frameln_act_bwd_fused_kernel", 4.0 * 3 * frames * PF)
     if sk:
         _reduce_partials(sk, ws, dw, db, L.npvp_frameln_act_bwd_reduce, L.npvp_frameln_act_bwd_reduce_job, "npvp_frameln_act_bwd_reduce",
@@ -1115,16 +1137,17 @@
     return dh, dw, db
 
 
-def _fln_pgrad(dout, h, mean, rstd, w, b, frames, PF, d, sk):
+def _fln_pgrad(dout, h, mean, rstd, w, b, frames, PF, d, sk, skip=NO_DROP, T=1):
+    sp, ss, sf = _skip_site(skip, T)
     L = lib()
     dev = h.device
     psum = torch.empty(frames * (PF // 1024) * 2, dtype=torch.float32, device=dev)
     dw, db = (sk[0][0], sk[1][0]) if sk else (torch.empty_like(w), torch.empty_like(b))
     ws, wsn = _ws(L.npvp_frameln_act_bwd_workspace_bytes(frames, PF), dev)
-    seed = _S._cur.rng.seed_tensor(dev) if d.on else None
+    seed = _S._cur.rng.seed_tensor(dev) if (d.on or sp > 0) else None
     check(L.npvp_frameln_act_bwd_pgrad(_ptr(dout), _ptr(h), mean, rstd, _ptr(w), _ptr(b), _ptr(psum), _ptr(dw), _ptr(db),
-                                       frames, PF, d.p, d.salt, 0.0, 0, 1, _ptr(seed), _sink_mode(sk), _ptr(ws), wsn, _stream()),
-          "npvp_frameln_act_bwd_pgrad")
+                                       frames, PF, d.p, d.salt, 0.0, 0, 1, sp, ss, sf, _ptr(seed), _sink_mode(sk), _ptr(ws), wsn,
+                                       _stream()), "npvp_frameln_act_bwd_pgrad")
     if sk:
         _reduce_partials(sk, ws, dw, db, L.npvp_frameln_act_bwd_reduce, L.npvp_frameln_act_bwd_reduce_job, "npvp_frameln_act_bwd_reduce",
                          (frames, PF, 1), True)
@@ -1286,10 +1309,11 @@
         dev = x.device
         dout = _c(dout)
         dh3, gn3w, gn3b = _fln_bwd(dout, h3, stats[4], stats[5], n3w, n3b, frames, 64 * Co, d3, dp, T, s_n3)
-        da2, gw2, gb2 = linear_bwd(dh3, a2, w2, True if has_b2 else None, s_fc2)
+        rskip = Drop._like(dp, 1, 64 * T, max(1, frames // max(1, T))) if dp.on else NO_DROP
+        da2, gw2, gb2 = linear_bwd(dh3, a2, w2, True if has_b2 else None, s_fc2, a_skip=rskip)
         fuse_n2 = MID_BWD_N2 and hid // 16 <= 256
         if fuse_n2:
-            psum2, gn2w, gn2b = _fln_pgrad(da2, h2, _row(stats, 2), _row(stats, 3), n2w, n2b, frames, 64 * hid, d2, s_n2)
+            psum2, gn2w, gn2b = _fln_pgrad(da2, h2, _row(stats, 2), _row(stats, 3), n2w, n2b, frames, 64 * hid, d2, s_n2, skip=dp, T=T)
         else:
             dh2, gn2w, gn2b = _fln_bwd(da2, h2, stats[2], stats[3], n2w, n2b, frames, 64 * hid, d2, NO_DROP, 1, s_n2,
                                           want_amax=False)
@@ -1322,15 +1346,17 @@
             gdww = torch.empty(hid, 1, 3, 3, dtype=torch.float32, device=dev)
             check(L.npvp_transpose(_ptr(dwtb), _ptr(gdww), 1, 9, hid, _stream()), "npvp_transpose")
             gdwb = dwtb[9]
-        dh1, gn1w, gn1b = _fln_bwd(da1, h1, stats[0], stats[1], n1w, n1b, frames, 64 * hid, NO_DROP, NO_DROP, 1, s_n1,
-                                      psum=psum, nparts=nparts)
+        dh1, gn1w, gn1b = _fln_bwd(da1, h1, stats[0], stats[1], n1w, n1b, frames, 64 * hid, NO_DROP, NO_DROP, T, s_n1,
+                                      psum=psum, nparts=nparts, skip=dp)
         del da1
-        dx, gw1, gb1 = linear_bwd(dh1, x, w1, True if has_b1 else None, s_fc1)
+        dx, gw1, gb1 = linear_bwd(dh1, x, w1, True if has_b1 else None, s_fc1, a_skip=rskip)
         return (dx, dout if has_res else None, gw1, gb1, gn1w, gn1b, gdww, gdwb, gn2w, gn2b, gw2, gb2, gn3w, gn3b,
                 None, None, None, None)
 
 
 MID_BWD_N2 = True
+
+DROP_PATH_SKIP = True
 
 
 def mlpdwbn_fused_supported(R, C, hid, Co, H, W):
```

Measured after the change: 8551 (median of 6 runs). About the same (+0.4%).
